# drowe67/pirip

Hardware: AMD Instinct MI355X
Metric: IQ Msamples/s demodulated (2-FSK Fs=240k Rs=10k); BER vs CPU ref (higher is better)
Workload: dtype f32; 1 GPU; BASELINE configs[1]: 2-FSK Fs=240k Rs=10k -p 24, batched synthetic u8 IQ, device-resident (fsk_demod -d equivalent); streams_per_gpu=16384

## Files before the change

include/pirip_hip.h:

```cpp
#ifndef PIRIP_HIP_H
#define PIRIP_HIP_H

#include <stddef.h>
#include <stdint.h>

#ifdef __cplusplus
extern "C" {
#endif

#define PIRIP_OK               0
#define PIRIP_ERR_BAD_ARG     (-1)
#define PIRIP_ERR_BAD_CONFIG  (-2)
#define PIRIP_ERR_NO_DEVICE   (-3)
#define PIRIP_ERR_HIP         (-4)
#define PIRIP_ERR_NOMEM       (-5)
#define PIRIP_ERR_UNSUPPORTED (-6)

#define PIRIP_IN_CU8_FSKDEMOD 0
#define PIRIP_IN_CU8_CSDR     1
#define PIRIP_IN_CS16         2
#define PIRIP_IN_CF32         3

#define PIRIP_MODE_M_MAX 4
#define PIRIP_FSK_DEFAULT_P 8
#define PIRIP_FSK_DEFAULT_NSYM 50
#define PIRIP_FDMDV_SCALE 750
#define PIRIP_STATS_PER_FRAME 10


typedef struct pirip_fsk_params {
    int Fs;
    int Rs;
    int M;
    int P;
    int Nsym;
    int est_min;
    int est_max;
    int freq_est_type;
    int tone_spacing;
    int in_format;
} pirip_fsk_params;

typedef struct pirip_fsk_info {
    int Ts, N, Nmem, Ndft, Nbits, nin_max, nstreams;
    int bytes_per_sample;
} pirip_fsk_info;

typedef struct pirip_hip_demod pirip_hip_demod;

int pirip_hip_create(const pirip_fsk_params *params, int nstreams, int device, pirip_hip_demod **out);

typedef struct pirip_fsk_recalled {
    int hann_denominator_ndft;
    float tc;
    float est_space_rs;
    float nin_threshold;
    int nin_step_div;
    float s16_scale;
    float u8d_offset;
    float u8d_scale;
    int ndft_rule;
    int sf_power;
} pirip_fsk_recalled;
void pirip_hip_recalled_defaults(pirip_fsk_recalled *r);
int pirip_hip_create_recalled(const pirip_fsk_params *params, const pirip_fsk_recalled *recalled, int nstreams, int device, pirip_hip_demod **out);
int pirip_hip_destroy(pirip_hip_demod *h);
int pirip_hip_get_info(const pirip_hip_demod *h, pirip_fsk_info *info);
#define PIRIP_KERNEL_GENERAL 0
#define PIRIP_KERNEL_WAVE 2
#define PIRIP_KERNEL_EXACT 4
#define PIRIP_KERNEL_BLOCK 3
int pirip_hip_get_kernel(const pirip_hip_demod *h);
int pirip_hip_set_exact_first_frame(pirip_hip_demod *h, int enable);
int pirip_hip_get_kernel_name(const pirip_hip_demod *h, char *buf, size_t n);
int pirip_hip_reset(pirip_hip_demod *h, void *hip_stream);
int pirip_hip_clear_estimators(pirip_hip_demod *h, void *hip_stream);

int pirip_hip_demod_batch(pirip_hip_demod *h,
                          const void *d_in, size_t in_stride_bytes, int64_t nsamp,
                          uint8_t *d_bits, size_t bits_stride,
                          float *d_rx_filt, size_t filt_stride,
                          float *d_stats, size_t stats_stride,
                          int32_t *d_nframes, int64_t *d_consumed,
                          int64_t max_frames, void *hip_stream);

typedef struct pirip_capture_report {
    int32_t segments;
    int32_t segment_frames;
    int32_t passes;
    int32_t segments_rerun;
    int64_t frames_demodulated;
} pirip_capture_report;
int pirip_hip_demod_capture(pirip_hip_demod *h, const void *d_in, int64_t nsamp, uint8_t *d_bits, float *d_rx_filt, float *d_stats,
                            int64_t max_frames, int64_t *nframes, int64_t *consumed, pirip_capture_report *report, void *hip_stream);
int pirip_hip_demod_capture_host(pirip_hip_demod *h, const void *in, int64_t nsamp, uint8_t *bits, float *rx_filt, float *stats,
                                 int64_t max_frames, int64_t *nframes, int64_t *consumed, pirip_capture_report *report);

int pirip_hip_demod_host(pirip_hip_demod *h, const void *in, int64_t nsamp,
                         uint8_t *bits, float *rx_filt, float *stats,
                         int64_t max_frames, int64_t *nframes, int64_t *consumed);
int pirip_hip_nin0(pirip_hip_demod *h);

int pirip_hip_set_bit_packing(pirip_hip_demod *h, int packed);

int pirip_hip_set_estimator_band_only(pirip_hip_demod *h, int enable);

int pirip_hip_set_burst_mode(pirip_hip_demod *h, int enable);

int pirip_hip_get_Sf(pirip_hip_demod *h, int s, float *Sf_host);
int pirip_hip_enable_eye(pirip_hip_demod *h, int enable);
int pirip_hip_get_eye(pirip_hip_demod *h, int s, int normalise, float *rx_eye, int *neyetr, int *neyesamp);
int pirip_hip_get_scalars(pirip_hip_demod *h, int s, float out8[8]);
typedef struct pirip_stream_state {
    int nin;
    float norm_rx_timing, ppm, snr_est, SNRest, EbNodB, v_est, f_est[4];
    float rx_sig_pow, rx_nse_pow;
} pirip_stream_state;
int pirip_hip_get_stream_state(pirip_hip_demod *h, int s, pirip_stream_state *out);
int pirip_hip_set_freq_est_limits(pirip_hip_demod *h, int est_min, int est_max);

typedef struct pirip_hip_decim pirip_hip_decim;

int pirip_hip_decim_create(int decimation, float transition_bw, int out_s16, int device,
                           pirip_hip_decim **out);
int pirip_hip_decim_destroy(pirip_hip_decim *d);
int pirip_hip_decim_taps(const pirip_hip_decim *d, float *taps, int *ntaps);
#define PIRIP_DECIM_EXACT   0
#define PIRIP_DECIM_FMA     1
#define PIRIP_DECIM_FMA_RAW 2
int pirip_hip_decim_set_arith(pirip_hip_decim *d, int mode);
int pirip_hip_decim_get_arith(const pirip_hip_decim *d);
int64_t pirip_hip_decim_nout(const pirip_hip_decim *d, int64_t n_in);
int pirip_hip_decim_batch(pirip_hip_decim *d, const uint8_t *d_in, size_t in_stride_bytes,
                          int64_t n_in, void *d_out, size_t out_stride_bytes, int nstreams,
                          void *hip_stream);

int pirip_hip_synth_cu8(int Fs, int Rs, int M, int nstreams,
                        const int32_t *f1_hz, int tone_spacing_hz, const int32_t *skip_samples,
                        const uint8_t *d_bits, size_t bits_stride, int64_t nsym,
                        uint8_t *d_out, size_t out_stride_bytes, int64_t nsamp,
                        float amp, float sigma, uint64_t seed, void *hip_stream);

#define PIRIP_RX_TRIAL_SYNC 0x1
#define PIRIP_RX_SYNC       0x2
#define PIRIP_RX_BITS       0x4
#define PIRIP_RX_BIT_ERRORS 0x8
#define PIRIP_LDPC_INFO_PER_CALL 10

typedef struct pirip_hip_ldpc pirip_hip_ldpc;
typedef struct pirip_ldpc_info {
    int n, k, bits_per_frame, data_bytes, nbits_per_call, max_iter, nstreams;
    char name[64];
} pirip_ldpc_info;

int pirip_hip_ldpc_create(const char *code_path, int M, int Nsym, int nstreams, int device, pirip_hip_ldpc **out);
int pirip_hip_ldpc_destroy(pirip_hip_ldpc *h);
int pirip_hip_ldpc_get_info(const pirip_hip_ldpc *h, pirip_ldpc_info *info);
int pirip_hip_ldpc_reset(pirip_hip_ldpc *h, void *hip_stream);
int pirip_hip_ldpc_get_llr_history(pirip_hip_ldpc *h, int s, uint16_t *host_llr);
int pirip_hip_ldpc_rx_batch(pirip_hip_ldpc *h, const float *d_rx_filt, size_t filt_stride, const int32_t *d_ncalls, int ncalls,
                            uint8_t *d_status, uint8_t *d_payload, int32_t *d_info, void *hip_stream);
int pirip_hip_fsk_ldpc_rx_batch(pirip_hip_demod *dem, pirip_hip_ldpc *h, const void *d_in, size_t in_stride_bytes, int64_t nsamp,
                                uint8_t *d_status, uint8_t *d_payload, int32_t *d_info, float *d_stats, size_t stats_stride,
                                int32_t *d_nframes, int64_t *d_consumed, int64_t max_frames, void *hip_stream);
int pirip_hip_fsk_ldpc_last_path(const pirip_hip_ldpc *h);
typedef struct pirip_chain_group {
    pirip_hip_demod *dem; pirip_hip_ldpc *ldpc;
    const void *d_in; uint8_t *d_status; uint8_t *d_payload; int32_t *d_info; float *d_stats; int32_t *d_nframes; int64_t *d_consumed;
} pirip_chain_group;
int pirip_hip_fsk_ldpc_rx_batch_groups(const pirip_chain_group *groups, int ngroups, size_t in_stride_bytes, int64_t nsamp, size_t stats_stride,
                                       int64_t max_frames, void *hip_stream);
int pirip_hip_ldpc_rx_host(pirip_hip_ldpc *h, const float *rx_filt, int ncalls, uint8_t *status, uint8_t *payload, int32_t *info);
int pirip_hip_ldpc_llr(pirip_hip_ldpc *h, const float *d_rx_filt, int ncalls, float *d_llr, void *hip_stream);
int pirip_hip_ldpc_decode_llr(pirip_hip_ldpc *h, const float *d_llr, int ncw, uint8_t *d_bits, int32_t *d_iter_pcc, void *hip_stream);

typedef struct pirip_hip_rx pirip_hip_rx;
int pirip_hip_rx_create(pirip_hip_demod *dem, pirip_hip_ldpc *ldpc, pirip_hip_decim *dec, int64_t block, pirip_hip_rx **out);
int pirip_hip_rx_destroy(pirip_hip_rx *rx);
int64_t pirip_hip_rx_max_frames(const pirip_hip_rx *rx);
int pirip_hip_rx_input(pirip_hip_rx *rx, void **d_block, size_t *stride_bytes);
int pirip_hip_rx_process(pirip_hip_rx *rx, uint8_t *d_bits, size_t bits_stride, float *d_rx_filt, size_t filt_stride,
                         uint8_t *d_status, uint8_t *d_payload, int32_t *d_info, float *d_stats, size_t stats_stride,
                         int32_t *d_nframes, void *hip_stream);
int pirip_hip_rx_push(pirip_hip_rx *rx, const void *d_in, size_t in_stride_bytes,
                      uint8_t *d_bits, size_t bits_stride, float *d_rx_filt, size_t filt_stride,
                      uint8_t *d_status, uint8_t *d_payload, int32_t *d_info, float *d_stats, size_t stats_stride,
                      int32_t *d_nframes, void *hip_stream);
int pirip_hip_rx_get_counters(pirip_hip_rx *rx, int64_t *consumed_total, int32_t *backlog);
int pirip_hip_rx_reset(pirip_hip_rx *rx, void *hip_stream);

typedef struct pirip_hip_chan pirip_hip_chan;
typedef struct pirip_chan_info {
    int Fs, D, ntaps, ntaps_padded, ninputs, nchan, out_s16, device;
} pirip_chan_info;
int pirip_hip_chan_create(int Fs, int decimation, float transition_bw, int out_s16, int ninputs, int nchan, const int32_t *chan_input,
                          const int32_t *chan_offset_hz, int device, pirip_hip_chan **out);
int pirip_hip_chan_destroy(pirip_hip_chan *ch);
int pirip_hip_chan_get_info(const pirip_hip_chan *ch, pirip_chan_info *info);
int pirip_hip_chan_taps(const pirip_hip_chan *ch, float *taps, int *ntaps);
int64_t pirip_hip_chan_nout(const pirip_hip_chan *ch, int64_t n_in);
int pirip_hip_chan_batch(pirip_hip_chan *ch, const uint8_t *d_in, size_t in_stride_bytes, int64_t n_in, int64_t t0,
                         void *d_out, size_t out_stride_bytes, void *hip_stream);
int pirip_hip_rx_create_chan(pirip_hip_demod *dem, pirip_hip_ldpc *ldpc, pirip_hip_chan *chan, int64_t block, pirip_hip_rx **out);

#define PIRIP_TX_CARRIER_OFF 0xFF
typedef struct pirip_hip_tx pirip_hip_tx;
typedef struct pirip_tx_info {
    int Fs, Rs, M, Ts, n, k, bits_per_frame, data_bytes, preamble_syms, frame_syms, nstreams, device;
} pirip_tx_info;
int pirip_hip_tx_create(const char *code_path, int Fs, int Rs, int M, int nstreams, int device, pirip_hip_tx **out);
int pirip_hip_tx_destroy(pirip_hip_tx *h);
int pirip_hip_tx_get_info(const pirip_hip_tx *h, pirip_tx_info *info);
int pirip_hip_tx_set_tones(pirip_hip_tx *h, const int32_t *f1_hz, int tone_spacing_hz);
int pirip_hip_tx_set_gaps(pirip_hip_tx *h, const int32_t *lead_syms, const int32_t *gap_syms);
int pirip_hip_tx_reset(pirip_hip_tx *h, void *hip_stream);
int64_t pirip_hip_tx_max_syms(const pirip_hip_tx *h, int max_rec);
int pirip_hip_tx_frame(pirip_hip_tx *h, const uint8_t *d_records, size_t rec_stride, const int32_t *d_nrec, int max_rec,
                       uint8_t *d_syms, size_t sym_stride, int64_t max_syms, int32_t *d_nsym, uint8_t *d_bits, size_t bits_stride,
                       void *hip_stream);
int pirip_hip_tx_modulate(pirip_hip_tx *h, const uint8_t *d_syms, size_t sym_stride, const int32_t *d_nsym, int64_t nsym,
                          int out_format, void *d_out, size_t out_stride_bytes, float amp, float sigma, uint64_t seed, void *hip_stream);
int pirip_hip_tx_records_to_iq(pirip_hip_tx *h, const uint8_t *d_records, size_t rec_stride, const int32_t *d_nrec, int max_rec,
                               int64_t nsym, int out_format, void *d_out, size_t out_stride_bytes, float amp, float sigma, uint64_t seed,
                               int32_t *d_nsym, void *hip_stream);

#define PIRIP_TX_REPEAT_MAX_FRAMES 100
int pirip_hip_tx_repeat_max_records(const pirip_hip_tx *h, int ncalls);
int pirip_hip_tx_repeat_records(pirip_hip_tx *h, const uint8_t *d_status, size_t status_stride, const uint8_t *d_payload, size_t payload_stride,
                                const int32_t *d_ncalls, int ncalls, int source_byte, uint8_t *d_records, size_t rec_stride, int max_rec,
                                int32_t *d_nrec, void *hip_stream);

#ifndef PIRIP_NO_CODEC2_SHIM
typedef struct { float real; float imag; } COMP;
#define MODE_M_MAX 4

struct MODEM_STATS;
struct FSK {
    int Ndft, Fs, N, Rs, Ts, Nmem, P, Nsym, Nbits, f1_tx, tone_spacing, mode;
    float tc;
    int est_min, est_max, est_space;
    float *hann_table;
    float *Sf;
    COMP phi_c[MODE_M_MAX];
    COMP *f_dc;
    void *fft_cfg;
    float norm_rx_timing;
    COMP tx_phase_c;
    float EbNodB;
    float f_est[MODE_M_MAX];
    float f2_est[MODE_M_MAX];
    int freq_est_type;
    float ppm, SNRest, v_est, rx_sig_pow, rx_nse_pow;
    int nin, burst_mode, lock_nin;
    struct MODEM_STATS *stats;
    int normalise_eye;
    void *pirip_priv;
};

// ... 114 lines not shown
```

pirip_amd/binding.py:

```python
import ctypes as C
import os
import subprocess

_HERE = os.path.dirname(os.path.abspath(__file__))
_LIB = os.environ.get("PIRIP_HIP_LIB") or os.path.join(_HERE, "lib", "libpirip_hip.so")

IN_CU8_FSKDEMOD, IN_CU8_CSDR, IN_CS16, IN_CF32 = 0, 1, 2, 3
STATS_PER_FRAME = 10


class PiripError(RuntimeError):
    pass


class FskParams(C.Structure):
    _fields_ = [("Fs", C.c_int), ("Rs", C.c_int), ("M", C.c_int), ("P", C.c_int), ("Nsym", C.c_int),
                ("est_min", C.c_int), ("est_max", C.c_int), ("freq_est_type", C.c_int),
                ("tone_spacing", C.c_int), ("in_format", C.c_int)]


class FskInfo(C.Structure):
    _fields_ = [("Ts", C.c_int), ("N", C.c_int), ("Nmem", C.c_int), ("Ndft", C.c_int), ("Nbits", C.c_int),
                ("nin_max", C.c_int), ("nstreams", C.c_int), ("bytes_per_sample", C.c_int)]

# ... 97 lines not shown
    L.pirip_hip_rx_reset.argtypes = [vp, vp]
    L.pirip_hip_rx_create_chan.argtypes = [vp, vp, vp, i64, C.POINTER(vp)]
    L.pirip_hip_chan_create.argtypes = [i32, i32, C.c_float, i32, i32, i32, vp, vp, i32, C.POINTER(vp)]
    L.pirip_hip_chan_destroy.argtypes = [vp]
    L.pirip_hip_chan_get_info.argtypes = [vp, C.POINTER(ChanInfo)]
    L.pirip_hip_chan_taps.argtypes = [vp, vp, C.POINTER(i32)]
    L.pirip_hip_chan_nout.restype = i64
    L.pirip_hip_chan_nout.argtypes = [vp, i64]
    L.pirip_hip_chan_batch.argtypes = [vp, vp, sz, i64, i64, vp, sz, vp]
    L.pirip_hip_tx_create.argtypes = [C.c_char_p, i32, i32, i32, i32, i32, C.POINTER(vp)]
    L.pirip_hip_tx_destroy.argtypes = [vp]
    L.pirip_hip_tx_get_info.argtypes = [vp, C.POINTER(TxInfo)]
    L.pirip_hip_tx_set_tones.argtypes = [vp, vp, i32]
    L.pirip_hip_tx_set_gaps.argtypes = [vp, vp, vp]
    L.pirip_hip_tx_reset.argtypes = [vp, vp]
    L.pirip_hip_tx_max_syms.restype = i64
    L.pirip_hip_tx_max_syms.argtypes = [vp, i32]
    L.pirip_hip_tx_frame.argtypes = [vp, vp, sz, vp, i32, vp, sz, i64, vp, vp, sz, vp]
    L.pirip_hip_tx_modulate.argtypes = [vp, vp, sz, vp, i64, i32, vp, sz, C.c_float, C.c_float, C.c_uint64, vp]
    L.pirip_hip_tx_records_to_iq.argtypes = [vp, vp, sz, vp, i32, i64, i32, vp, sz, C.c_float, C.c_float, C.c_uint64, vp, vp]
    L.pirip_hip_tx_repeat_max_records.argtypes = [vp, i32]
    L.pirip_hip_tx_repeat_records.argtypes = [vp, vp, sz, vp, sz, vp, i32, i32, vp, sz, i32, vp, vp]
    _lib = L
    return L


def device_count():
    return int(lib().pirip_hip_device_count())


def selftest_sqrt():
    L = lib()
    m = C.c_uint64(0)
    L.pirip_hip_selftest_sqrt.argtypes = [C.POINTER(C.c_uint64)]
    _chk(L.pirip_hip_selftest_sqrt(C.byref(m)), "pirip_hip_selftest_sqrt")
    return int(m.value)


def selftest_div():
    L = lib()
    m = C.c_uint64(0)
    L.pirip_hip_selftest_div.argtypes = [C.POINTER(C.c_uint64)]
    _chk(L.pirip_hip_selftest_div(C.byref(m)), "pirip_hip_selftest_div")
    return int(m.value)


def _chk(rc, what):
    if rc != 0:
        raise PiripError(f"{what}: {lib().pirip_hip_strerror(rc).decode()} ({rc})")


class FskRecalled(C.Structure):
    _fields_ = [("hann_denominator_ndft", C.c_int), ("tc", C.c_float), ("est_space_rs", C.c_float), ("nin_threshold", C.c_float),
                ("nin_step_div", C.c_int), ("s16_scale", C.c_float), ("u8d_offset", C.c_float), ("u8d_scale", C.c_float),
                ("ndft_rule", C.c_int), ("sf_power", C.c_int)]


def recalled(**overrides):
    r = FskRecalled()
    lib().pirip_hip_recalled_defaults(C.byref(r))
    for k, v in overrides.items():
        if k not in dict(FskRecalled._fields_):
            raise KeyError(k)
        setattr(r, k, v)
    return r


class HipDemod:

    def __init__(self, Fs, Rs, M, P=8, Nsym=50, est_min=0, est_max=0, mask=0, in_format=IN_CU8_FSKDEMOD,
                 nstreams=1, device=-1, recalled=None):
        self.L = lib()
        self.params = FskParams(Fs, Rs, M, P, Nsym, est_min, est_max, 1 if mask else 0, mask if mask else 100, in_format)
        h = C.c_void_p()
        if recalled is None:
            _chk(self.L.pirip_hip_create(C.byref(self.params), nstreams, device, C.byref(h)), "pirip_hip_create")
        else:
            rc = globals()["recalled"](**recalled)
            _chk(self.L.pirip_hip_create_recalled(C.byref(self.params), C.byref(rc), nstreams, device, C.byref(h)), "pirip_hip_create_recalled")
        self.h = h
        self.info = FskInfo()
        _chk(self.L.pirip_hip_get_info(self.h, C.byref(self.info)), "pirip_hip_get_info")
        self.nstreams = nstreams
        self.M, self.Nsym, self.Nbits, self.N = M, Nsym, self.info.Nbits, self.info.N

    def close(self):
        if getattr(self, "h", None):
            self.L.pirip_hip_destroy(self.h)
            self.h = None

    __del__ = close

    def kernel(self):
        self.L.pirip_hip_get_kernel.argtypes = [C.c_void_p]
        k = self.L.pirip_hip_get_kernel(self.h)
        return "wave" if k == 2 else "block" if k == 3 else "exact" if k == 4 else "general"

    def kernel_name(self):
        buf = C.create_string_buffer(256)
        self.L.pirip_hip_get_kernel_name.argtypes = [C.c_void_p, C.c_char_p, C.c_size_t]
        _chk(self.L.pirip_hip_get_kernel_name(self.h, buf, 256), "pirip_hip_get_kernel_name")
        return buf.value.decode()

    def reset(self, stream=0):
        _chk(self.L.pirip_hip_reset(self.h, stream), "pirip_hip_reset")

    def max_frames_for(self, nsamp):
        return nsamp // (2 * self.N - self.info.nin_max) + 2

    def demod_batch(self, d_in, in_stride, nsamp, d_bits=0, bits_stride=0, d_filt=0, filt_stride=0,
                    d_stats=0, stats_stride=0, d_nframes=0, d_consumed=0, max_frames=None, stream=0):
        if max_frames is None:
            max_frames = self.max_frames_for(nsamp)
        _chk(self.L.pirip_hip_demod_batch(self.h, d_in, in_stride, nsamp, d_bits, bits_stride, d_filt, filt_stride,
                                          d_stats, stats_stride, d_nframes, d_consumed, max_frames, stream),
             "pirip_hip_demod_batch")

    def demod_capture(self, d_in, nsamp, d_bits, d_filt=0, d_stats=0, max_frames=None, stream=0):
        if max_frames is None:
            max_frames = self.max_frames_for(nsamp)
        nf, cons, rep = C.c_int64(0), C.c_int64(0), CaptureReport()
        _chk(self.L.pirip_hip_demod_capture(self.h, d_in, nsamp, d_bits, d_filt, d_stats, max_frames, C.byref(nf), C.byref(cons),
                                            C.byref(rep), stream), "pirip_hip_demod_capture")
        return nf.value, cons.value, {k: getattr(rep, k) for k, _ in CaptureReport._fields_}

    def demod_host(self, buf, want_filt=True):
        import numpy as np
        buf = np.ascontiguousarray(buf)
        nsamp = buf.shape[0]
        maxf = self.max_frames_for(nsamp)
        fb = (self.Nbits + 7) // 8 if getattr(self, "packed", False) else self.Nbits
        bits = np.zeros((maxf, fb), dtype=np.uint8)
        filt = np.zeros((maxf, self.M * self.Nsym), dtype=np.float32)
        st = np.zeros((maxf, STATS_PER_FRAME), dtype=np.float32)
        nf, cons = C.c_int64(0), C.c_int64(0)
        _chk(self.L.pirip_hip_demod_host(self.h, buf.ctypes.data, nsamp, bits.ctypes.data,
                                         filt.ctypes.data if want_filt else None, st.ctypes.data, maxf,
                                         C.byref(nf), C.byref(cons)), "pirip_hip_demod_host")
        n = nf.value
        return {"nframes": n, "consumed": cons.value, "bits": bits[:n], "rx_filt": filt[:n] if want_filt else None,
                "stats": st[:n]}

    def set_bit_packing(self, packed=True):
        _chk(self.L.pirip_hip_set_bit_packing(self.h, 1 if packed else 0), "pirip_hip_set_bit_packing")
        self.packed = bool(packed)

    def set_exact_first_frame(self, enable=True):
        self.L.pirip_hip_set_exact_first_frame.argtypes = [C.c_void_p, C.c_int]
        _chk(self.L.pirip_hip_set_exact_first_frame(self.h, 1 if enable else 0), "pirip_hip_set_exact_first_frame")

    def set_estimator_band_only(self, enable=True):
        _chk(self.L.pirip_hip_set_estimator_band_only(self.h, 1 if enable else 0), "pirip_hip_set_estimator_band_only")

    def set_freq_est_limits(self, est_min, est_max):
        return int(self.L.pirip_hip_set_freq_est_limits(self.h, int(est_min), int(est_max)))

    def set_burst_mode(self, enable=True):
        _chk(self.L.pirip_hip_set_burst_mode(self.h, 1 if enable else 0), "pirip_hip_set_burst_mode")

    def enable_eye(self, enable=True):
        self.L.pirip_hip_enable_eye.argtypes = [C.c_void_p, C.c_int]
        _chk(self.L.pirip_hip_enable_eye(self.h, 1 if enable else 0), "pirip_hip_enable_eye")

    def eye(self, s=0, normalise=True):
        import numpy as np
        out = np.zeros((8, 160), dtype=np.float32)
        ntr, npt = C.c_int(0), C.c_int(0)
        self.L.pirip_hip_get_eye.argtypes = [C.c_void_p, C.c_int, C.c_int, C.c_void_p, C.c_void_p, C.c_void_p]
        _chk(self.L.pirip_hip_get_eye(self.h, s, 1 if normalise else 0, out.ctypes.data, C.byref(ntr), C.byref(npt)), "pirip_hip_get_eye")
        return out[:ntr.value, :npt.value].copy()

    def get_Sf(self, s=0):
        import numpy as np
        out = np.zeros(self.info.Ndft, dtype=np.float32)
        _chk(self.L.pirip_hip_get_Sf(self.h, s, out.ctypes.data), "pirip_hip_get_Sf")
        return out


class HipDecim:

    def __init__(self, D, transition_bw=0.05, out_s16=True, device=-1):
        self.L = lib()
        h = C.c_void_p()
        _chk(self.L.pirip_hip_decim_create(D, transition_bw, 1 if out_s16 else 0, device, C.byref(h)),
             "pirip_hip_decim_create")
        self.h, self.D, self.out_s16 = h, D, out_s16

    def close(self):
        if getattr(self, "h", None):
            self.L.pirip_hip_decim_destroy(self.h)
            self.h = None

    __del__ = close

    def taps(self):
        import numpy as np
        n = C.c_int(0)
        self.L.pirip_hip_decim_taps(self.h, None, C.byref(n))
        t = np.zeros(n.value, dtype=np.float32)
        self.L.pirip_hip_decim_taps(self.h, t.ctypes.data, C.byref(n))
        return t

    def nout(self, n_in):
        return int(self.L.pirip_hip_decim_nout(self.h, n_in))

    def set_arith(self, mode):
        _chk(self.L.pirip_hip_decim_set_arith(self.h, int(mode)), "pirip_hip_decim_set_arith")

    def batch(self, d_in, in_stride, n_in, d_out, out_stride, nstreams, stream=0):
        _chk(self.L.pirip_hip_decim_batch(self.h, d_in, in_stride, n_in, d_out, out_stride, nstreams, stream),
             "pirip_hip_decim_batch")


class HipChan:

    def __init__(self, Fs, D, offsets, inputs=None, transition_bw=0.05, out_s16=False, device=-1):
        import numpy as np
        self.L = lib()
        off = np.ascontiguousarray(offsets, dtype=np.int32).reshape(-1)
        inp = np.zeros(off.size, dtype=np.int32) if inputs is None else np.ascontiguousarray(inputs, dtype=np.int32).reshape(-1)
        if inp.size != off.size:
            raise ValueError("inputs and offsets must have the same length")
        ninputs = int(inp.max()) + 1 if inp.size else 1
        h = C.c_void_p()
        _chk(self.L.pirip_hip_chan_create(int(Fs), int(D), transition_bw, 1 if out_s16 else 0, ninputs, int(off.size),
                                          inp.ctypes.data if inp.size else None, off.ctypes.data if off.size else None, device, C.byref(h)),
             "pirip_hip_chan_create")
        self.h = h
        self.info = ChanInfo()
        _chk(self.L.pirip_hip_chan_get_info(self.h, C.byref(self.info)), "pirip_hip_chan_get_info")
        self.Fs, self.D, self.out_s16 = int(Fs), int(D), bool(out_s16)
        self.offsets, self.inputs = off.copy(), inp.copy()
        self.ninputs, self.nchan, self.Lp = self.info.ninputs, self.info.nchan, self.info.ntaps_padded
        self.bytes_per_sample = 4 if out_s16 else 8

    def close(self):
        if getattr(self, "h", None):
            self.L.pirip_hip_chan_destroy(self.h)
            self.h = None

    __del__ = close

    def taps(self):
        import numpy as np
        n = C.c_int(0)
        self.L.pirip_hip_chan_taps(self.h, None, C.byref(n))
        t = np.zeros(n.value, dtype=np.float32)
        self.L.pirip_hip_chan_taps(self.h, t.ctypes.data, C.byref(n))
        return t

    def nout(self, n_in):
        return int(self.L.pirip_hip_chan_nout(self.h, int(n_in)))

    def batch(self, d_in, in_stride, n_in, d_out, out_stride, t0=0, stream=0):
        _chk(self.L.pirip_hip_chan_batch(self.h, d_in, in_stride, int(n_in), int(t0), d_out, out_stride, stream), "pirip_hip_chan_batch")


TX_CARRIER_OFF = 0xFF


class HipTx:

    def __init__(self, code_path, Fs, Rs, M, nstreams=1, f1=None, shift=None, lead=0, gap=0, device=-1):
        self.L = lib()
        h = C.c_void_p()
        _chk(self.L.pirip_hip_tx_create(code_path.encode(), int(Fs), int(Rs), int(M), int(nstreams), device, C.byref(h)), "pirip_hip_tx_create")
        self.h = h
        self.info = TxInfo()
        _chk(self.L.pirip_hip_tx_get_info(self.h, C.byref(self.info)), "pirip_hip_tx_get_info")
        self.Fs, self.Rs, self.M, self.Ts, self.nstreams = int(Fs), int(Rs), int(M), self.info.Ts, int(nstreams)
        self.k, self.data_bytes, self.record_bytes = self.info.k, self.info.data_bytes, 1 + self.info.data_bytes
        self.bits_per_frame, self.frame_syms, self.preamble_syms = self.info.bits_per_frame, self.info.frame_syms, self.info.preamble_syms
        self.bps = 1 if M == 2 else 2
        if f1 is not None:
            self.set_tones(f1, shift if shift is not None else Rs)
        self.set_gaps(lead, gap)

    def close(self):
        if getattr(self, "h", None):
            self.L.pirip_hip_tx_destroy(self.h)
            self.h = None

    __del__ = close

    def _per_stream(self, v):
        import numpy as np
        a = np.ascontiguousarray(v, dtype=np.int32).reshape(-1)
        if a.size == 1:
            a = np.full(self.nstreams, int(a[0]), dtype=np.int32)
        if a.size != self.nstreams:
            raise ValueError("one value, or one per stream")
        return a

    def set_tones(self, f1, shift):
        a = self._per_stream(f1)
        _chk(self.L.pirip_hip_tx_set_tones(self.h, a.ctypes.data, int(shift)), "pirip_hip_tx_set_tones")

    def set_gaps(self, lead=0, gap=0):
        a, b = self._per_stream(lead), self._per_stream(gap)
        _chk(self.L.pirip_hip_tx_set_gaps(self.h, a.ctypes.data, b.ctypes.data), "pirip_hip_tx_set_gaps")

    def reset(self, stream=0):
        _chk(self.L.pirip_hip_tx_reset(self.h, stream), "pirip_hip_tx_reset")

    def max_syms(self, max_rec):
        return int(self.L.pirip_hip_tx_max_syms(self.h, int(max_rec)))
# ... 158 lines not shown
```

pirip_amd/csrc/demod_handle.hpp:

```cpp
#pragma once
#include <hip/hip_runtime.h>
#include <cstdint>

#include "fsk_device.hpp"
#include "fsk_plan.hpp"

struct CaptureWork;

struct pirip_hip_demod {
    pirip::FskPlan plan;
    int nstreams = 0;
    int device = 0;
    int last_hip = 0;
    int kernel = 0;
    float *d_hann = nullptr; float2 *d_tw = nullptr; uint16_t *d_perm = nullptr; float *d_lut = nullptr;
    float2 *d_tph = nullptr; int16_t *d_teeth = nullptr; uint32_t *d_mask_dtheta = nullptr;
    float2 *d_osc_drift = nullptr; float2 *d_osc_step = nullptr; float2 *d_timing_rec = nullptr; float *d_fast_tab = nullptr;
    float *d_Sf = nullptr; uint32_t *d_theta = nullptr; float2 *d_hist = nullptr; pirip::StreamScalars *d_scal = nullptr; float2 *d_phic = nullptr;
    void *d_stage_in = nullptr; size_t stage_in_bytes = 0;
    uint8_t *d_stage_bits = nullptr; float *d_stage_filt = nullptr; float *d_stage_stats = nullptr;
    int32_t *d_stage_nframes = nullptr; int64_t *d_stage_consumed = nullptr; int64_t stage_frames = 0;
    int nin0 = 0;
    bool fresh = true;
    int exact0 = 1;
    int32_t *d_first = nullptr;
    float *d_eye = nullptr;
    struct CaptureWork *capture = nullptr;
};

namespace pirip {
void demod_fill_args(const pirip_hip_demod *h, DemodArgs *a);
bool demod_bind(const pirip_hip_demod *h);
}
```

pirip_amd/csrc/fsk_demod_wave.hip:

```cpp
#include <hip/hip_runtime.h>

#include <cmath>
#include <cstdio>
#include <cstdlib>

#include "../../include/pirip_hip.h"
#include "demod_simd.hpp"
#include "fsk_device.hpp"

namespace pirip {

namespace {

constexpr int kWave = 64;

struct cf { float x, y; };

__device__ __forceinline__ float add_lane_up(float a, float b)
{
    float r;
    asm("v_add_f32_dpp %0, %1, %2 wave_shl:1 row_mask:0xf bank_mask:0xf bound_ctrl:0" : "=v"(r) : "v"(a), "v"(b));
    return r;
}

// ... 28 lines not shown

__device__ __forceinline__ v2f scale_lo(v2f h, v2f x)
{
    v2f r; asm("v_pk_mul_f32 %0, %1, %2 op_sel_hi:[0,1]" : "=v"(r) : "v"(h), "v"(x)); return r;
}
__device__ __forceinline__ v2f scale_hi(v2f h, v2f x)
{
    v2f r; asm("v_pk_mul_f32 %0, %1, %2 op_sel:[1,0] op_sel_hi:[1,1]" : "=v"(r) : "v"(h), "v"(x)); return r;
}
__device__ __forceinline__ float mag2(v2f w)
{
    v2f sq;
    asm("v_pk_mul_f32 %0, %1, %1" : "=v"(sq) : "v"(w));
    float r;
    asm("v_add_f32 %0, %1, %2" : "=v"(r) : "v"(sq.x), "v"(sq.y));
    return r;
}
__device__ __forceinline__ v2f smooth2(v2f sf, v2f mag, v2f k)
{
    v2f t;
    asm("v_pk_mul_f32 %0, %0, %3 op_sel_hi:[1,0]\n\t"
        "v_pk_mul_f32 %1, %2, %3 op_sel:[0,1] op_sel_hi:[1,1]\n\t"
        "v_pk_add_f32 %0, %0, %1"
        : "+v"(sf), "=&v"(t) : "v"(mag), "v"(k));
    return sf;
}

template <int FMT> struct InFmt;
template <> struct InFmt<PIRIP_IN_CU8_FSKDEMOD> { static constexpr int BPS = 2; static constexpr bool NEUTRAL_OK = true; static constexpr uint32_t NEUTRAL = 0x7F7F7F7Fu; };
template <> struct InFmt<PIRIP_IN_CU8_CSDR> { static constexpr int BPS = 2; static constexpr bool NEUTRAL_OK = false; static constexpr uint32_t NEUTRAL = 0x80808080u; };
template <> struct InFmt<PIRIP_IN_CS16> { static constexpr int BPS = 4; static constexpr bool NEUTRAL_OK = true; static constexpr uint32_t NEUTRAL = 0u; };
template <> struct InFmt<PIRIP_IN_CF32> { static constexpr int BPS = 8; static constexpr bool NEUTRAL_OK = true; static constexpr uint32_t NEUTRAL = 0u; };

__device__ __forceinline__ float cvt_s16(float x)
{
    const float hi = x * 0.00133514404296875f;
    return __builtin_fmaf(x, -0x1.e60f04p-20f, hi);
}
template <int FMT>
__device__ __forceinline__ v2f decode(const uint32_t *rw, int k)
{
    if (FMT == PIRIP_IN_CU8_FSKDEMOD || FMT == PIRIP_IN_CU8_CSDR) {
        const uint32_t v = rw[k >> 1];
        return cvt_u8_pair<FMT>(v2f{(k & 1) ? ubyte2(v) : ubyte0(v), (k & 1) ? ubyte3(v) : ubyte1(v)});
    } else if (FMT == PIRIP_IN_CS16) {
        const uint32_t v = rw[k];
        return v2f{cvt_s16((float)(short)(v & 0xffffu)), cvt_s16((float)((int)v >> 16))};
    } else {
        return v2f{__builtin_bit_cast(float, rw[2 * k]), __builtin_bit_cast(float, rw[2 * k + 1])};
    }
}
template <int FMT>
__device__ __forceinline__ v2f lds_sample(const unsigned char *p)
{
    if (FMT == PIRIP_IN_CU8_FSKDEMOD || FMT == PIRIP_IN_CU8_CSDR) {
        const uint32_t v = *(const uint16_t *)p;
        return cvt_u8_pair<FMT>(v2f{ubyte0(v), ubyte1(v)});
    } else if (FMT == PIRIP_IN_CS16) {
        const uint32_t v = *(const uint32_t *)p;
        return v2f{cvt_s16((float)(short)(v & 0xffffu)), cvt_s16((float)((int)v >> 16))};
    } else {
        const float2 v = *(const float2 *)p;
        return v2f{v.x, v.y};
    }
}

constexpr int cmax(int a, int b) { return a > b ? a : b; }

__device__ __forceinline__ float atan2_turns(float y, float x)
{
    const float ax = fabsf(x), ay = fabsf(y);
    const float mn = ax < ay ? ax : ay, mx = ax < ay ? ay : ax;
    const float t = mx > 0.f ? mn * __builtin_amdgcn_rcpf(mx) : 0.f;
    const float s1 = t * t, s2 = s1 * s1, s4 = s2 * s2;
    const float p01 = __builtin_fmaf(s1, -0.05304612219333649f, 0.15915483236312866f);
    const float p23 = __builtin_fmaf(s1, -0.02213626727461815f, 0.031745944172143936f);
    const float p45 = __builtin_fmaf(s1, -0.00889870710670948f, 0.015346021391451359f);
    const float p67 = __builtin_fmaf(s1, -0.0006453014793805778f, 0.0034795869141817093f);
    const float q0 = __builtin_fmaf(s2, p23, p01), q1 = __builtin_fmaf(s2, p67, p45);
    float r = __builtin_fmaf(s4, q1, q0) * t;
    r = ay > ax ? 0.25f - r : r;
    r = x < 0.f ? 0.5f - r : r;
    return __builtin_copysignf(r, y);
}

constexpr float kLlrMax = 24.0f;
__device__ __forceinline__ float ln_i0_tab(const float *tab, float x)
{
    const bool in = x < 32.0f;
    const float xs = (in ? x : 32.0f) * 8.0f;
    const int j = (int)xs;
    const float f = xs - (float)j;
    const float t0 = tab[j], t1 = tab[j + 1];
    return (t0 + (f * (t1 - t0))) + (in ? 0.0f : x - 32.0f);
}
__device__ __forceinline__ uint32_t spread16(uint32_t x)
{
    x = (x | (x << 8)) & 0x00FF00FFu; x = (x | (x << 4)) & 0x0F0F0F0Fu; x = (x | (x << 2)) & 0x33333333u; x = (x | (x << 1)) & 0x55555555u;
    return x;
}

#ifdef PIRIP_WAVE_TIMING
__device__ int g_wave_stop_phase = -1;
#define PIRIP_T_DECL long long t_acc_[8] = {0, 0, 0, 0, 0, 0, 0, 0}; long long t_last_ = __builtin_amdgcn_s_memtime(); \
    const int t_stop_ = __builtin_amdgcn_readfirstlane(g_wave_stop_phase)
#define PIRIP_T_MARK(i) { const long long t_now_ = __builtin_amdgcn_s_memtime(); t_acc_[i] += t_now_ - t_last_; t_last_ = t_now_; } \
    if (t_stop_ == (i)) { pos += nin; frame++; wave_lds_sync(); continue; } else (void)0
#else
#define PIRIP_T_DECL do { } while (0)
#define PIRIP_T_MARK(i) do { } while (0)
#endif

template <int M, int TS, int P, int NSYM, int NDFT, int FMT>
struct WaveCfg {
    static constexpr int BPS = InFmt<FMT>::BPS;
    static constexpr int N = TS * NSYM;
    static constexpr int NMEM = N + 2 * TS;
    static constexpr int Q = TS / 4;
    static constexpr int HIST = 2 * TS + Q;
    static constexpr int STEP = TS / P;
    static constexpr int NLANES = NSYM + 2;
    static constexpr int NFFT = (N - Q) / (NDFT / 2) - 1;
    static constexpr int GUARD_B = ((HIST * BPS + 15) / 16) * 16;
    static constexpr int SUP_B = (N + Q) * BPS;
    static constexpr int NDMA16 = SUP_B / 1024;
    static constexpr int NDMA4 = (SUP_B - NDMA16 * 1024 + 255) / 256;
    static constexpr bool DIRECT = FMT == PIRIP_IN_CF32 && NDFT >= 256;
    static constexpr int HEAD_B = 1024, DUMP_B = 256;
    static_assert(!DIRECT || ((TS + Q) * BPS <= HEAD_B && 3 * TS >= 2 * TS + Q), "the head holds blocks 0..2's new samples");
    static constexpr int RAW_B = DIRECT ? GUARD_B + HEAD_B + DUMP_B : GUARD_B + NDMA16 * 1024 + NDMA4 * 256;
    static constexpr int XPS256 = 16 * 17 * 8;
    static constexpr int XP_FFT_B = NDFT == 256 ? 4 * XPS256 : NDFT == 512 ? 4480 : 8 * 72 * 8;
    static constexpr int XP_B = cmax(cmax(XP_FFT_B, NDFT * 4), NDFT == 256 ? 64 * 20 * 4 : NDFT == 128 ? 8 * 136 * 4 : 0);
    static constexpr int TAIL_DW = HIST * BPS / 4;
    static constexpr int TRAILER_DW = GUARD_B / 4;
    static_assert((HIST * BPS) % 4 == 0 && (GUARD_B - HIST * BPS) % 4 == 0, "tail copies move whole dwords");
    static_assert(GUARD_B + (2 * M + 1) * 4 <= M * HIST * 8, "the state block holds the raw tail and its trailer");
    static constexpr int CHS = (BPS == 2) ? TS : (TS % 8 == 0 ? 8 : TS % 4 == 0 ? 4 : 2);
    static constexpr int CH_DW = CHS * BPS / 4;
    static_assert(TS % 2 == 0 && TS % P == 0 && P >= 4, "bad Ts / P");
    static_assert(NLANES <= kWave, "one lane per symbol block");
    static_assert((TS * BPS) % 16 == 0 && (CHS * BPS) % 16 == 0 && TS % CHS == 0, "block and chunk strides keep 16-byte alignment");
    static_assert((N + Q) / (NDFT / 2) - 1 == NFFT && N / (NDFT / 2) - 1 == NFFT, "numffts must not depend on nin");
    static_assert(NDFT == 256 ? (NFFT >= 4) : NDFT == 512 ? (NFFT % 2 == 0) : (NDFT == 128 && NFFT <= 8),
                  "FFT batches (Ndft = 256: the last batch of 4 may be partial; Ndft = 128: one batch of up to eight)");
    static_assert((NFFT - 1) * (NDFT / 2) + NDFT <= N - Q, "FFT windows stay inside the shortest frame");
    static_assert(M * P <= 48, "window prefix sums are kept in registers");
};

template <class C, int M> constexpr int wave_lds_bytes() { return C::RAW_B + C::XP_B; }

}

template <int M, int TS, int P, int NSYM, int NDFT, int FMT, int WPB, int WPS, bool FFT_FMA = false, bool MASK = false, int BAND = 0>
__global__ __launch_bounds__(kWave * WPB, WPS) void fsk_demod_wave_kernel(DemodArgs a_kernarg, int nstreams)
{
    constexpr bool INPLACE = TS == 10;
    static_assert(offsetof(DemodArgs, d) == 0, "the argument block is the first kernel argument");
    auto ap = [&]() {
        if constexpr (INPLACE) return (const __attribute__((address_space(4))) DemodArgs *)__builtin_amdgcn_kernarg_segment_ptr();
        else return (const DemodArgs *)&a_kernarg;
    }();
#define PIRIP_ARGS_REREAD() do { if constexpr (INPLACE) asm volatile("" : "+s"(ap)); } while (0)
#define a (*ap)
#define d (ap->d)
    static_assert(BAND == 0 || ((BAND == 2 || BAND == 4) && NDFT == 256 && !MASK), "band-only estimator: Ndft = 256, peak method, 32 or 64 bins");
    auto cmul = [](v2f x, v2f t) { return FFT_FMA ? rot_step(x, t) : cmul_x(x, t); };
    using C = WaveCfg<M, TS, P, NSYM, NDFT, FMT>;
    constexpr int N = C::N, NMEM = C::NMEM, HIST = C::HIST, STEP = C::STEP, Q = C::Q, BPS = C::BPS;
    constexpr int GUARD_B = C::GUARD_B;

    __shared__ __attribute__((aligned(16))) unsigned char s_raw[WPB][C::RAW_B];
    __shared__ __attribute__((aligned(16))) unsigned char s_xp[WPB][C::XP_B];
    constexpr int TAB_F = NDFT == 256 ? 12 * 16 * 4 : NDFT == 512 ? 8 * 16 * 2 + 12 * 32 * 2 : 8 * 16 * 2;
    __shared__ __attribute__((aligned(16))) float s_tab[TAB_F];
    __shared__ __attribute__((aligned(16))) float2 s_tph[P];
    __shared__ __attribute__((aligned(16))) float2 s_tgain[NSYM + 2];
    __shared__ float s_misc[WPB][3];
    extern __shared__ __attribute__((aligned(16))) float s_lnI0[];

    const int lane0 = threadIdx.x & (kWave - 1);
    const int wv = __builtin_amdgcn_readfirstlane(threadIdx.x >> 6);
    const int sid = blockIdx.x * WPB + wv;

    if (NDFT == 256) {
        for (int i = threadIdx.x; i < 12 * 16; i += kWave * WPB)
            ((float4 *)s_tab)[i] = ((const float4 *)a.t.fast_tab)[(i & 15) * 12 + (i >> 4)];
    } else {
        for (int i = threadIdx.x; i < TAB_F / 4; i += kWave * WPB) ((float4 *)s_tab)[i] = ((const float4 *)(a.t.fast_tab + NDFT))[i];
    }
    if constexpr (P <= 10) if (a.io.soft.llr) {
        if (a.io.soft.llr_map == kLlrRician) { for (int i = threadIdx.x; i < 258; i += kWave * WPB) s_lnI0[i] = a.io.soft.lnI0[i]; }
        else if (threadIdx.x < 20) {
            const int sg = threadIdx.x >> 2, cc = threadIdx.x & 3;
            const float c2 = sg == 0 ? 0.226f : sg == 1 ? 0.1245f : sg == 2 ? 0.0288f : sg == 3 ? 0.002f : 0.0f;
            const float c1 = sg == 0 ? 0.0125f : sg == 1 ? 0.2177f : sg == 2 ? 0.6314f : sg == 3 ? 0.9048f : 0.9867f;
            const float c0 = sg == 0 ? -0.0012f : sg == 1 ? -0.108f : sg == 2 ? -0.5645f : sg == 3 ? -1.2997f : -2.2053f;
            s_lnI0[threadIdx.x] = cc == 0 ? c2 : cc == 1 ? c1 : cc == 2 ? c0 : 0.0f;
        }
    }
    if (threadIdx.x < P) s_tph[threadIdx.x] = a.t.tph[threadIdx.x];
    if (threadIdx.x < NSYM + 2) s_tgain[threadIdx.x] = a.t.timing_rec[(threadIdx.x < NSYM + 1 ? threadIdx.x : 0) * P];
    __syncthreads();
    if (sid >= nstreams) return;
    if (a.io.seg && a.io.seg[sid].max_frames < 0) return;

    unsigned char *raw = s_raw[wv];
    unsigned char *xpb = s_xp[wv];

    uint32_t *st32 = (uint32_t *)(a.s.hist + (size_t)sid * M * HIST);
    int ninp = __builtin_amdgcn_readfirstlane((int)st32[C::TRAILER_DW + 2 * M]);
    uint32_t dthp[M];
    int tixp[M];
#pragma unroll
    for (int m = 0; m < M; m++) {
        dthp[m] = (uint32_t)__builtin_amdgcn_readfirstlane((int)st32[C::TRAILER_DW + m]);
        tixp[m] = __builtin_amdgcn_readfirstlane((int)st32[C::TRAILER_DW + M + m]);
    }
    for (int i = lane0; i < GUARD_B / 4; i += kWave) ((uint32_t *)raw)[i] = ninp ? st32[i] : InFmt<FMT>::NEUTRAL;

#define PIRIP_PHASE_LANE(name) int name = lane0; asm volatile("" : "+v"(name))
    constexpr int NOWN = NDFT / kWave;
    constexpr int NB = BAND ? BAND : NOWN;
    auto own_sfi = [](int ln, int b) {
        const int bin = BAND ? ((ln & 15) + 16 * b)
                      : NDFT == 256 ? ((ln & 15) + 16 * b + 64 * (ln >> 4)) : NDFT == 512 ? ((ln & 31) + 32 * (8 * (ln >> 5) + b)) : (ln + 64 * b);
        return (bin + NDFT / 2) & (NDFT - 1);
    };
    float Sf[NOWN];
    float hann16[NDFT == 256 ? 1 : 16];
    if constexpr (NDFT == 512) {
#pragma unroll
        for (int i = 0; i < 16; i++) hann16[i] = a.t.fast_tab[(lane0 & 31) + 32 * (i >> 3) + 64 * (i & 7)];
    }
    if constexpr (NDFT == 128) {
#pragma unroll
        for (int i = 0; i < 16; i++) hann16[i] = a.t.fast_tab[(lane0 & 7) + 8 * i];
    }
#pragma unroll
    for (int b = 0; b < NB; b++) Sf[b] = a.s.Sf[(size_t)sid * NDFT + own_sfi(lane0, b)];

    float sc_norm_rx_timing, sc_ppm, sc_SNRest;
    int sc_nin;
    {
        const StreamScalars sc = a.s.scal[sid];
        sc_norm_rx_timing = sc.norm_rx_timing; sc_ppm = sc.ppm; sc_SNRest = sc.SNRest; sc_nin = sc.nin;
        if (lane0 == 0) { s_misc[wv][0] = sc.snr_est; s_misc[wv][1] = sc.EbNodB; s_misc[wv][2] = sc.v_est; }
    }

    int64_t seg_in = 0, out0 = 0, max_frames = a.io.max_frames;
    if (a.io.seg) {
        const SegDesc sd = a.io.seg[sid];
        seg_in = sd.in_off; out0 = sd.out_frame0; max_frames = sd.max_frames;
    }
    const uint8_t *in_base = a.io.in + (size_t)sid * a.io.in_stride + (size_t)seg_in * BPS;
    const int64_t nsamp = a.io.nsamp - seg_in;
    const __amdgpu_buffer_rsrc_t rsrc =
        __builtin_amdgcn_make_buffer_rsrc((void *)in_base, 0, (int)(uint32_t)(BPS * nsamp), 0x00020000);

    int nin = __builtin_amdgcn_readfirstlane(sc_nin);
    int64_t pos = 0, frame = 0;
    if (a.io.first) { pos = __builtin_amdgcn_readfirstlane(a.io.first[sid]); frame = pos ? 1 : 0; }
    const int64_t frame_first = frame;
    int last_freqi0 = 0, last_freqi1 = 0, last_freqi2 = 0, last_freqi3 = 0;

    typedef __attribute__((address_space(3))) void *lds_ptr;
    auto dma_frame = [&](int64_t p0) {
        const uint32_t goff = (uint32_t)__builtin_amdgcn_readfirstlane((int)(uint32_t)(p0 * BPS));
        if constexpr (C::DIRECT) {
            __builtin_amdgcn_raw_ptr_buffer_load_lds(rsrc, (lds_ptr)(raw + GUARD_B), 16, lane0 * 16, goff, 0, 0);
#pragma unroll
            for (int i = 0; i < (C::SUP_B + 8191) / 8192; i++)
                __builtin_amdgcn_raw_ptr_buffer_load_lds(rsrc, (lds_ptr)(raw + GUARD_B + C::HEAD_B), 4, lane0 * 128, goff + i * 8192, 0, 0);
            return;
        }
#pragma unroll
        for (int i = 0; i < C::NDMA16; i++)
            __builtin_amdgcn_raw_ptr_buffer_load_lds(rsrc, (lds_ptr)(raw + GUARD_B + i * 1024), 16, lane0 * 16, goff + i * 1024, 0, 0);
#pragma unroll
        for (int i = 0; i < C::NDMA4; i++)
            __builtin_amdgcn_raw_ptr_buffer_load_lds(rsrc, (lds_ptr)(raw + GUARD_B + C::NDMA16 * 1024 + i * 256), 4, lane0 * 4,
                                                     goff + C::NDMA16 * 1024 + i * 256, 0, 0);
    };
    constexpr bool SOFT_OK = P <= 10;
    uint32_t soft_carry = 0;
    int soft_cb = 0, soft_w = 0;
    uint32_t *words_o = nullptr;
    if constexpr (SOFT_OK) if (a.io.soft.llr) { words_o = a.io.soft.words + (size_t)sid * a.io.soft.words_stride + (a.io.soft.bit0 >> 5); }
    auto soft_append = [&](uint32_t W, int nb) {
        const uint32_t merged = soft_carry | (soft_cb ? (W >> soft_cb) : W);
        if (soft_cb + nb >= 32) {
            if (lane0 == 0) words_o[soft_w] = merged;
            soft_w++;
            soft_carry = soft_cb ? (W << (32 - soft_cb)) : 0u;
            soft_cb = soft_cb + nb - 32;
        } else { soft_carry = merged; soft_cb += nb; }
    };
    constexpr int NBITS = NSYM * (M == 2 ? 1 : 2);
    wave_lds_sync();
    dma_frame(pos);
    PIRIP_T_DECL;

    while (frame < max_frames && pos + nin <= nsamp) {
        PIRIP_ARGS_REREAD();
        const int nold = NMEM - nin;
        PIRIP_T_MARK(7);
        asm volatile("s_waitcnt vmcnt(0)" ::: "memory");
        wave_lds_sync();
        PIRIP_T_MARK(0);
        const unsigned char *smp = raw + GUARD_B;
        const uint32_t goff_frame = (uint32_t)__builtin_amdgcn_readfirstlane((int)(uint32_t)(pos * BPS));
        auto fft_in = [&](const unsigned char *p) -> v2f {
            if constexpr (C::DIRECT && BPS == 8) {
                const auto v = __builtin_amdgcn_raw_buffer_load_b64(rsrc, (int)(p - smp), (int)goff_frame, 0);
                return __builtin_bit_cast(v2f, v);
            } else if constexpr (C::DIRECT) {
                const uint32_t v = (uint32_t)__builtin_amdgcn_raw_buffer_load_b32(rsrc, (int)(p - smp), (int)goff_frame, 0);
                return v2f{cvt_s16((float)(short)(v & 0xffffu)), cvt_s16((float)((int)v >> 16))};
            } else return lds_sample<FMT>(p);
        };
        const v2f ktc{d.one_minus_tc, d.tc};
        if constexpr (NDFT == 256) {
            PIRIP_PHASE_LANE(lane);
            const int grp = lane >> 4, e16 = lane & 15;
            const float4 *ftab = (const float4 *)s_tab + e16;
            constexpr int XPS = C::XPS256;
            float4 tabv[12];
#pragma unroll
            for (int i = 0; i < 12; i++) tabv[i] = ftab[16 * i];
#pragma unroll 1
            for (int bt = 0; bt < (C::NFFT + 3) / 4; bt++) {
                int jj = 4 * bt + grp;
                if (C::NFFT % 4) jj = jj < C::NFFT ? jj : C::NFFT - 1;
                const int ga = e16 >> 2, gb = e16 & 3;
                const int base = ga + 4 * gb;
                const unsigned char *src = smp + BPS * ((NDFT / 2) * jj + base);
                v2f W[16];
                v2f hann2[8];
                {
                    const float4 h0 = tabv[0], h1 = tabv[1], h2 = tabv[2], h3 = tabv[3];
                    hann2[0] = v2f{h0.x, h0.y}; hann2[1] = v2f{h0.z, h0.w}; hann2[2] = v2f{h1.x, h1.y}; hann2[3] = v2f{h1.z, h1.w};
                    hann2[4] = v2f{h2.x, h2.y}; hann2[5] = v2f{h2.z, h2.w}; hann2[6] = v2f{h3.x, h3.y}; hann2[7] = v2f{h3.z, h3.w};
                }
#pragma unroll
                for (int t = 0; t < 16; t++) {
                    const v2f x = fft_in(src + 16 * BPS * t);
                    const int c = t & 3, dd = t >> 2;
                    W[4 * c + dd] = (t & 1) ? scale_hi(hann2[t >> 1], x) : scale_lo(hann2[t >> 1], x);
                }
#pragma unroll
                for (int c = 0; c < 4; c++) bfly4(W[4 * c], W[4 * c + 1], W[4 * c + 2], W[4 * c + 3]);
                bfly4(W[0], W[4], W[8], W[12]);
#pragma unroll
                for (int k = 1; k < 4; k++) {
                    v2f f1 = cmul(W[4 + k], v2f{a.tw_s2[6 * (k - 1) + 0], a.tw_s2[6 * (k - 1) + 1]});
                    v2f f2 = cmul(W[8 + k], v2f{a.tw_s2[6 * (k - 1) + 2], a.tw_s2[6 * (k - 1) + 3]});
                    v2f f3 = cmul(W[12 + k], v2f{a.tw_s2[6 * (k - 1) + 4], a.tw_s2[6 * (k - 1) + 5]});
                    bfly4(W[k], f1, f2, f3);
                    W[4 + k] = f1; W[8 + k] = f2; W[12 + k] = f3;
                }
                {
                    float2 *xp = (float2 *)(xpb + grp * XPS);
#pragma unroll
                    for (int e = 0; e < 16; e++) xp[e16 * 17 + e] = make_float2(W[e].x, W[e].y);
                    wave_lds_sync();
#pragma unroll
                    for (int g = 0; g < 16; g++) { const float2 v = xp[g * 17 + e16]; W[g] = v2f{v.x, v.y}; }
                }
                {
                    const float4 c4 = tabv[4], c5 = tabv[5];
                    const v2f tw3[3] = {v2f{c4.x, c4.y}, v2f{c4.z, c4.w}, v2f{c5.x, c5.y}};
#pragma unroll
                    for (int aa = 0; aa < 4; aa++) {
                        v2f f1 = cmul(W[4 * aa + 1], tw3[0]);
                        v2f f2 = cmul(W[4 * aa + 2], tw3[1]);
                        v2f f3 = cmul(W[4 * aa + 3], tw3[2]);
                        bfly4(W[4 * aa], f1, f2, f3);
                        W[4 * aa + 1] = f1; W[4 * aa + 2] = f2; W[4 * aa + 3] = f3;
                    }
                }
#pragma unroll
                for (int b = 0; b < (BAND ? BAND : 4); b++) {
                    const float *trow = (const float *)(ftab);
                    auto tf = [&](int f) { const float4 c = tabv[f >> 2]; return (f & 3) == 0 ? c.x : (f & 3) == 1 ? c.y : (f & 3) == 2 ? c.z : c.w; };
                    (void)trow;
                    const v2f t1{tf(22 + 6 * b), tf(23 + 6 * b)}, t2{tf(24 + 6 * b), tf(25 + 6 * b)}, t3{tf(26 + 6 * b), tf(27 + 6 * b)};
                    v2f f1 = cmul(W[4 + b], t1);
                    v2f f2 = cmul(W[8 + b], t2);
                    v2f f3 = cmul(W[12 + b], t3);
                    bfly4(W[b], f1, f2, f3);
                    W[4 + b] = f1; W[8 + b] = f2; W[12 + b] = f3;
                }
                wave_lds_sync();
                if constexpr (BAND != 0) {
                    float m2b[BAND], rb[BAND];
                    unsigned kmin = 0xffffffffu;
#pragma unroll
                    for (int b = 0; b < BAND; b++) { m2b[b] = mag2(W[b]); kmin = umin2(kmin, fbits(m2b[b])); }
                    if (__all(kmin >= kSqrtLo)) {
#pragma unroll
                        for (int b = 0; b < BAND; b++) rb[b] = sqrt_rn_normal<FMT != PIRIP_IN_CF32, true>(m2b[b]);
                    } else {
                        kmin = 0xffffffffu;
#pragma unroll
                        for (int b = 0; b < BAND; b++) kmin = umin2(kmin, sqrt_key(m2b[b]));
                        if (__all(kmin >= kSqrtLo - 1u)) {
#pragma unroll
                            for (int b = 0; b < BAND; b++) rb[b] = sqrt_rn_normal<FMT != PIRIP_IN_CF32>(m2b[b]);
                        } else {
#pragma unroll
                            for (int b = 0; b < BAND; b++) rb[b] = sqrtf(m2b[b]);
                        }
                    }
                    float2 *mx = (float2 *)xpb;
#pragma unroll
                    for (int b = 0; b < BAND; b += 2) mx[(b / 2) * 64 + lane] = make_float2(rb[b], rb[b + 1]);
                    wave_lds_sync();
                    float2 rt[BAND / 2][4];
#pragma unroll
                    for (int b = 0; b < BAND; b += 2)
#pragma unroll
                        for (int g2 = 0; g2 < 4; g2++) rt[b / 2][g2] = mx[(b / 2) * 64 + g2 * 16 + e16];
#pragma unroll
                    for (int b = 0; b < BAND; b += 2) {
                        v2f sp{Sf[b], Sf[b + 1]};
#pragma unroll
                        for (int g2 = 0; g2 < 4; g2++)
                            if (C::NFFT % 4 == 0 || 4 * bt + g2 < C::NFFT) sp = smooth2(sp, v2f{rt[b / 2][g2].x, rt[b / 2][g2].y}, ktc);
                        Sf[b] = sp.x; Sf[b + 1] = sp.y;
                    }
                    wave_lds_sync();
                } else {
                    float *mx = (float *)xpb;
                    float4 *row = (float4 *)(mx + lane * 20);
#pragma unroll
                    for (int q4 = 0; q4 < 4; q4++)
                        row[q4] = make_float4(mag2(W[4 * q4 + 0]), mag2(W[4 * q4 + 1]), mag2(W[4 * q4 + 2]), mag2(W[4 * q4 + 3]));
                    wave_lds_sync();
                    float4 m2[4];
                    unsigned kmin = 0xffffffffu;
#pragma unroll
                    for (int g2 = 0; g2 < 4; g2++) {
                        m2[g2] = *(const float4 *)(mx + (g2 * 16 + e16) * 20 + 4 * grp);
                        kmin = umin3(umin3(kmin, fbits(m2[g2].x), fbits(m2[g2].y)), fbits(m2[g2].z), fbits(m2[g2].w));
                    }
                    float4 rt[4];
                    if (__all(kmin >= kSqrtLo)) {
#pragma unroll
                        for (int g2 = 0; g2 < 4; g2++)
                            rt[g2] = make_float4(sqrt_rn_normal<FMT != PIRIP_IN_CF32, true>(m2[g2].x), sqrt_rn_normal<FMT != PIRIP_IN_CF32, true>(m2[g2].y),
                                                 sqrt_rn_normal<FMT != PIRIP_IN_CF32, true>(m2[g2].z), sqrt_rn_normal<FMT != PIRIP_IN_CF32, true>(m2[g2].w));
                    } else {
                        kmin = 0xffffffffu;
#pragma unroll
                        for (int g2 = 0; g2 < 4; g2++)
                            kmin = umin3(umin3(kmin, sqrt_key(m2[g2].x), sqrt_key(m2[g2].y)), sqrt_key(m2[g2].z), sqrt_key(m2[g2].w));
                        if (__all(kmin >= kSqrtLo - 1u)) {
#pragma unroll
                            for (int g2 = 0; g2 < 4; g2++)
                                rt[g2] = make_float4(sqrt_rn_normal<FMT != PIRIP_IN_CF32>(m2[g2].x), sqrt_rn_normal<FMT != PIRIP_IN_CF32>(m2[g2].y),
                                                     sqrt_rn_normal<FMT != PIRIP_IN_CF32>(m2[g2].z), sqrt_rn_normal<FMT != PIRIP_IN_CF32>(m2[g2].w));
                        } else {
#pragma unroll
                            for (int g2 = 0; g2 < 4; g2++) {
                                rt[g2] = make_float4(sqrtf(m2[g2].x), sqrtf(m2[g2].y), sqrtf(m2[g2].z), sqrtf(m2[g2].w));
                                __builtin_amdgcn_sched_barrier(0);
                            }
                        }
                    }
                    {
                        v2f s01{Sf[0], Sf[1]}, s23{Sf[2], Sf[3]};
#pragma unroll
                        for (int g2 = 0; g2 < 4; g2++) {
                            if (C::NFFT % 4 == 0 || 4 * bt + g2 < C::NFFT) {
                                s01 = smooth2(s01, v2f{rt[g2].x, rt[g2].y}, ktc);
                                s23 = smooth2(s23, v2f{rt[g2].z, rt[g2].w}, ktc);
                            }
                        }
                        Sf[0] = s01.x; Sf[1] = s01.y; Sf[2] = s23.x; Sf[3] = s23.y;
                    }
                    wave_lds_sync();
                }
            }
        } else if constexpr (NDFT == 128) {
            PIRIP_PHASE_LANE(lane);
            const int f8 = lane >> 3, l8 = lane & 7;
            const int jj = f8 < C::NFFT ? f8 : C::NFFT - 1;
            const float2 *s_p2 = (const float2 *)s_tab;
            float2 *xf = (float2 *)xpb + f8 * 72;
            v2f V[16];
            {
                const unsigned char *src = smp + BPS * ((NDFT / 2) * jj + l8);
#pragma unroll
                for (int u = 0; u < 2; u++) {
                    v2f S[8];
                    {
                        v2f Wt[8];
#pragma unroll
                        for (int t = 0; t < 8; t++) {
                            const int y = u + 2 * (t & 3) + 8 * (t >> 2);
                            const v2f x = fft_in(src + BPS * 8 * y);
                            const float hn = hann16[y];
                            Wt[t] = v2f{hn * x.x, hn * x.y};
                        }
#pragma unroll
                        for (int q2 = 0; q2 < 4; q2++) { S[2 * q2] = Wt[q2] + Wt[q2 + 4]; S[2 * q2 + 1] = Wt[q2] - Wt[q2 + 4]; }
                    }
                    bfly4(S[0], S[2], S[4], S[6]);
                    {
                        v2f f1 = cmul(S[3], v2f{a.tw_s2[0], a.tw_s2[1]});
                        v2f f2 = cmul(S[5], v2f{a.tw_s2[2], a.tw_s2[3]});
                        v2f f3 = cmul(S[7], v2f{a.tw_s2[4], a.tw_s2[5]});
                        bfly4(S[1], f1, f2, f3);
                        S[3] = f1; S[5] = f2; S[7] = f3;
                    }
                    if (u == 1) wave_lds_sync();
                    float2 *wr = xf + l8 * 9;
#pragma unroll
                    for (int r = 0; r < 8; r++) wr[r] = make_float2(S[r].x, S[r].y);
                    wave_lds_sync();
#pragma unroll
                    for (int q0 = 0; q0 < 4; q0++)
#pragma unroll
                        for (int ql = 0; ql < 2; ql++) { const float2 v = xf[(q0 + 4 * ql) * 9 + l8]; V[4 * q0 + 2 * u + ql] = v2f{v.x, v.y}; }
                }
            }
            {
                const float2 t1 = s_p2[l8 * 16 + 0], t2 = s_p2[l8 * 16 + 1], t3 = s_p2[l8 * 16 + 2];
#pragma unroll
                for (int q0 = 0; q0 < 4; q0++) {
                    v2f f1 = cmul(V[4 * q0 + 1], v2f{t1.x, t1.y});
                    v2f f2 = cmul(V[4 * q0 + 2], v2f{t2.x, t2.y});
                    v2f f3 = cmul(V[4 * q0 + 3], v2f{t3.x, t3.y});
                    bfly4(V[4 * q0], f1, f2, f3);
                    V[4 * q0 + 1] = f1; V[4 * q0 + 2] = f2; V[4 * q0 + 3] = f3;
                }
            }
#pragma unroll
            for (int j1 = 0; j1 < 4; j1++) {
                const float2 t1 = s_p2[l8 * 16 + 3 + 3 * j1], t2 = s_p2[l8 * 16 + 4 + 3 * j1], t3 = s_p2[l8 * 16 + 5 + 3 * j1];
                v2f f1 = cmul(V[4 + j1], v2f{t1.x, t1.y});
                v2f f2 = cmul(V[8 + j1], v2f{t2.x, t2.y});
                v2f f3 = cmul(V[12 + j1], v2f{t3.x, t3.y});
                bfly4(V[j1], f1, f2, f3);
                V[4 + j1] = f1; V[8 + j1] = f2; V[12 + j1] = f3;
            }
            wave_lds_sync();
            {
                float *mx = (float *)xpb;
#pragma unroll
                for (int i = 0; i < 16; i++) mx[f8 * 136 + l8 + 8 * i] = mag2(V[i]);
                wave_lds_sync();
                float A[C::NFFT], B[C::NFFT];
                unsigned kmin = 0xffffffffu;
#pragma unroll
                for (int j = 0; j < C::NFFT; j++) {
                    A[j] = mx[j * 136 + lane]; B[j] = mx[j * 136 + lane + 64];
                    kmin = umin3(kmin, fbits(A[j]), fbits(B[j]));
                }
                if (__all(kmin >= kSqrtLo)) {
#pragma unroll
                    for (int j = 0; j < C::NFFT; j++) { A[j] = sqrt_rn_normal<FMT != PIRIP_IN_CF32, true>(A[j]); B[j] = sqrt_rn_normal<FMT != PIRIP_IN_CF32, true>(B[j]); }
                } else {
                    kmin = 0xffffffffu;
#pragma unroll
                    for (int j = 0; j < C::NFFT; j++) kmin = umin3(kmin, sqrt_key(A[j]), sqrt_key(B[j]));
                    if (__all(kmin >= kSqrtLo - 1u)) {
#pragma unroll
                        for (int j = 0; j < C::NFFT; j++) { A[j] = sqrt_rn_normal<FMT != PIRIP_IN_CF32>(A[j]); B[j] = sqrt_rn_normal<FMT != PIRIP_IN_CF32>(B[j]); }
                    } else {
#pragma unroll
                        for (int j = 0; j < C::NFFT; j++) { A[j] = sqrtf(A[j]); B[j] = sqrtf(B[j]); __builtin_amdgcn_sched_barrier(0); }
                    }
                }
                v2f sp{Sf[0], Sf[1]};
#pragma unroll
                for (int j = 0; j < C::NFFT; j++) sp = smooth2(sp, v2f{A[j], B[j]}, ktc);
                Sf[0] = sp.x; Sf[1] = sp.y;
                wave_lds_sync();
            }
        } else {
            PIRIP_PHASE_LANE(lane);
            const int hh = lane >> 5, L5 = lane & 31;
            const float2 *s_p2 = (const float2 *)s_tab;
            const float2 *s_p3 = (const float2 *)(s_tab + 8 * 16 * 2);
            const int q0w = L5 & 3, q1w = (L5 >> 2) & 3, q2w = L5 >> 4;
            const int q0r = L5 >> 3, r2 = L5 & 7;
            float2 *x1 = (float2 *)xpb + hh * 280;
            float2 *x2 = (float2 *)xpb + hh * 160;
#pragma unroll 1
            for (int bt = 0; bt < C::NFFT / 2; bt++) {
                const int jj = 2 * bt + hh;
                const unsigned char *src = smp + BPS * ((NDFT / 2) * jj + L5);
                v2f V[16];
#pragma unroll
                for (int u = 0; u < 2; u++) {
                    v2f S[8];
                    {
                        v2f Wt[8];
#pragma unroll
                        for (int t = 0; t < 8; t++) {
                            const v2f x = fft_in(src + BPS * (32 * u + 64 * t));
                            const float hn = hann16[8 * u + t];
                            Wt[t] = v2f{hn * x.x, hn * x.y};
                        }
#pragma unroll
                        for (int q3 = 0; q3 < 4; q3++) { S[2 * q3] = Wt[q3] + Wt[q3 + 4]; S[2 * q3 + 1] = Wt[q3] - Wt[q3 + 4]; }
                    }
                    bfly4(S[0], S[2], S[4], S[6]);
                    {
                        v2f f1 = cmul(S[3], v2f{a.tw_s2[0], a.tw_s2[1]});
                        v2f f2 = cmul(S[5], v2f{a.tw_s2[2], a.tw_s2[3]});
                        v2f f3 = cmul(S[7], v2f{a.tw_s2[4], a.tw_s2[5]});
                        bfly4(S[1], f1, f2, f3);
                        S[3] = f1; S[5] = f2; S[7] = f3;
                    }
                    if (u == 1) wave_lds_sync();
                    {
                        float2 *wr = x1 + (q0w * 9 + q1w * 2 + q2w) * 8;
#pragma unroll
                        for (int r = 0; r < 8; r++) wr[r ^ q1w] = make_float2(S[r].x, S[r].y);
                    }
                    wave_lds_sync();
#pragma unroll
                    for (int q1 = 0; q1 < 4; q1++)
#pragma unroll
                        for (int q2l = 0; q2l < 2; q2l++) {
                            const float2 v = x1[(q0r * 9 + q1 * 2 + q2l) * 8 + (r2 ^ q1)];
                            V[4 * q1 + 2 * u + q2l] = v2f{v.x, v.y};
                        }
                }
                {
                    const float2 t1 = s_p2[r2 * 16 + 0], t2 = s_p2[r2 * 16 + 1], t3 = s_p2[r2 * 16 + 2];
// ... 351 lines not shown
                    if (low_sample >= 0) { lo[m].x = lane_up(lo[m].x); lo[m].y = lane_up(lo[m].y); }
                    if (high_sample >= 0) { hi[m].x = lane_up(hi[m].x); hi[m].y = lane_up(hi[m].y); }
                }
            }
            float tmax[M];
            float sum = 0.f;
#pragma unroll
            for (int m = 0; m < M; m++) {
                v2f t;
                t.x = (1 - fract) * lo[m].x; t.y = (1 - fract) * lo[m].y;
                t.x = t.x + fract * hi[m].x; t.y = t.y + fract * hi[m].y;
                tmax[m] = (t.x * t.x) + (t.y * t.y);
                sum += tmax[m];
            }
            float mx = tmax[0]; int sym = 0;
#pragma unroll
            for (int m = 1; m < M; m++) if (tmax[m] > mx) { mx = tmax[m]; sym = m; }
            const bool act = lane < NSYM;
            if (bits_o && !d.pack_bits) {
                if (act) {
                    if (M == 2) bits_o[lane] = sym == 1;
                    else { bits_o[2 * lane + 1] = sym & 1; bits_o[2 * lane] = (sym & 2) >> 1; }
                }
            } else if (bits_o) {
                const unsigned long long mlo = __ballot(act && (sym & 1)), mhi = __ballot(act && (sym & 2));
                if (lane < frame_bytes) {
                    unsigned byte = 0;
                    if (M == 2) {
                        byte = __builtin_bitreverse32((unsigned)(mlo >> (8 * lane)) & 0xffu) >> 24;
                    } else {
                        const unsigned h4 = (unsigned)(mhi >> (4 * lane)) & 0xfu, l4 = (unsigned)(mlo >> (4 * lane)) & 0xfu;
#pragma unroll
                        for (int q = 0; q < 4; q++) byte |= (((h4 >> q) & 1u) << (7 - 2 * q)) | (((l4 >> q) & 1u) << (6 - 2 * q));
                    }
                    bits_o[lane] = (uint8_t)byte;
                }
            }
            if (act && filt_o) {
#pragma unroll
                for (int m = 0; m < M; m++) filt_o[m * NSYM + lane] = sqrtf(tmax[m]);
            }
            if constexpr (SOFT_OK) if (a.io.soft.llr) {
                float mag[M], sum2 = 0.f, mx2 = 0.f;
                unsigned kmin = 0xffffffffu, kmax = 0u;
#pragma unroll
                for (int m = 0; m < M; m++) { kmin = umin2(kmin, sqrt_key(tmax[m])); kmax = kmax > fbits(tmax[m]) ? kmax : fbits(tmax[m]); }
                const bool quick = __all(!act || (kmin >= 0x0f800000u - 1u && kmax <= kQuickHi));
                float ssig, snse;
                if (quick) {
#pragma unroll
                    for (int m = 0; m < M; m++) { mag[m] = sqrt_rn_normal<FMT != PIRIP_IN_CF32>(tmax[m]); const float p2 = mag[m] * mag[m]; sum2 = sum2 + p2; mx2 = p2 > mx2 ? p2 : mx2; }
                    ssig = wave_sum(act ? mx2 : 0.f); snse = wave_sum(act ? div_rn_const<M - 1>(sum2 - mx2) : 0.f);
                    ssig = div_rn_const<NSYM>(ssig);
                    snse = div_rn_const<NSYM>(snse) + 1e-12f;
                } else {
#pragma unroll
                    for (int m = 0; m < M; m++) { mag[m] = sqrtf(tmax[m]); const float p2 = mag[m] * mag[m]; sum2 = sum2 + p2; mx2 = p2 > mx2 ? p2 : mx2; }
                    ssig = wave_sum(act ? mx2 : 0.f); snse = wave_sum(act ? (sum2 - mx2) / (float)(M - 1) : 0.f);
                    ssig = ssig / (float)NSYM;
                    snse = (snse / (float)NSYM) + 1e-12f;
                }
                const int llr_map = a.io.soft.llr_map;
                const float g = llr_frame_gain_quick(llr_map, ssig, snse);
                float L[M];
                if (llr_map == kLlrRician) {
#pragma unroll
                    for (int m = 0; m < M; m++) L[m] = ln_i0_tab(s_lnI0, g * mag[m]);
                } else {
#pragma unroll
                    for (int m = 0; m < M; m++) {
                        const float x = g * mag[m];
                        int sg = x >= 1.0f ? 1 : 0;
                        sg = x >= 2.0f ? 2 : sg; sg = x >= 5.0f ? 3 : sg; sg = x >= 20.0f ? 4 : sg;
                        const float4 cf = ((const float4 *)s_lnI0)[sg];
                        L[m] = (((cf.x * x) * x) + (cf.y * x)) + cf.z;
                    }
                }
                float l0, l1 = 0.f;
                if (M == 2) l0 = L[0] - L[M - 1];
                else {
                    l0 = (L[0] > L[1] ? L[0] : L[1]) - (L[M - 2] > L[M - 1] ? L[M - 2] : L[M - 1]);
                    l1 = (L[0] > L[M - 2] ? L[0] : L[M - 2]) - (L[1] > L[M - 1] ? L[1] : L[M - 1]);
                }
                const float lmax = llr_map == kLlrRician ? kLlrMax : kLlrMaxUpstream;
                l0 = l0 > lmax ? lmax : (l0 < -lmax ? -lmax : l0);
                l1 = l1 > lmax ? lmax : (l1 < -lmax ? -lmax : l1);
                const _Float16 h0v = (_Float16)l0, h1v = (_Float16)l1;
                l0 = (float)h0v; l1 = (float)h1v;
                uint16_t *llr_o = a.io.soft.llr + (size_t)sid * a.io.soft.llr_stride + a.io.soft.bit0 + (size_t)frame * NBITS;
                if (act) {
                    if (M == 2) llr_o[lane] = __builtin_bit_cast(uint16_t, h0v);
                    else *(uint32_t *)(llr_o + 2 * lane) = (uint32_t)__builtin_bit_cast(uint16_t, h0v) | ((uint32_t)__builtin_bit_cast(uint16_t, h1v) << 16);
                }
                const unsigned long long h0 = __ballot(act && l0 < 0.0f), h1 = __ballot(act && l1 < 0.0f);
                if (M == 2) {
                    soft_append(__builtin_bitreverse32((uint32_t)h0), 32);
                    soft_append(__builtin_bitreverse32((uint32_t)(h0 >> 32)), NBITS - 32);
                } else {
#pragma unroll
                    for (int j = 0; j < (NBITS + 31) / 32; j++) {
                        const uint32_t z = spread16((uint32_t)(h0 >> (16 * j)) & 0xffffu) | (spread16((uint32_t)(h1 >> (16 * j)) & 0xffffu) << 1);
                        soft_append(__builtin_bitreverse32(z), (j + 1) * 32 <= NBITS ? 32 : NBITS - 32 * j);
                    }
                }
            }
            const bool last_frame = (frame + 1 >= max_frames) || (pos + nin + nin_next > nsamp);
            if (stats_o || last_frame) {
                float sig = act ? mx : 0.f, nse = act ? (sum - mx) / (float)(M - 1) : 0.f;
                sig = wave_sum(sig); nse = wave_sum(nse) + 1e-12f;
                sig = sig / (float)NSYM; nse = nse / (float)NSYM;
                sc_SNRest = sig / nse;
                float mean_e = wave_sum(act ? sqrtf(mx) : 0.f), std_e = wave_sum(act ? mx : 0.f);
                mean_e = mean_e / (float)NSYM;
                std_e = (std_e / (float)NSYM) - (mean_e * mean_e);
                std_e = std_e > 0.0f ? sqrtf(std_e) : 0.0f;
                const float EbNodB = -6.0f + (20.0f * log10f((1e-6f + mean_e) / (1e-6f + std_e)));
                if (lane == 0) {
                    s_misc[wv][0] = (0.5f * s_misc[wv][0]) + (0.5f * EbNodB);
                    s_misc[wv][1] = EbNodB;
                    s_misc[wv][2] = sqrtf(sig - nse);
                    a.s.scal[sid].rx_sig_pow = sig; a.s.scal[sid].rx_nse_pow = nse;
                    if (stats_o) { stats_o[8] = sig; stats_o[9] = nse; }
                }
            }
        } else {
            for (int i = lane; i < frame_bytes; i += kWave) if (bits_o) bits_o[i] = 0;
            for (int i = lane; i < M * NSYM; i += kWave) if (filt_o) filt_o[i] = 0.f;
            if (stats_o && lane == 0) { stats_o[8] = 0.f; stats_o[9] = 0.f; }
            if constexpr (SOFT_OK) if (a.io.soft.llr) {
                uint16_t *llr_o = a.io.soft.llr + (size_t)sid * a.io.soft.llr_stride + a.io.soft.bit0 + (size_t)frame * NBITS;
                for (int i = lane; i < NBITS; i += kWave) llr_o[i] = 0;
                for (int j = 0; j < (NBITS + 31) / 32; j++) soft_append(0u, (j + 1) * 32 <= NBITS ? 32 : NBITS - 32 * j);
            }
        }
        if constexpr (MASK) last_freqi0 = bb;
        else { last_freqi0 = freqi[0]; last_freqi1 = freqi[M > 1 ? 1 : 0]; last_freqi2 = freqi[M > 2 ? 2 : 0]; last_freqi3 = freqi[M > 3 ? 3 : 0]; }
        if (stats_o && lane == 0) {
            stats_o[0] = f_est[0]; stats_o[1] = f_est[1]; stats_o[2] = f_est[2]; stats_o[3] = f_est[3];
            stats_o[4] = sc_norm_rx_timing; stats_o[5] = sc_SNRest; stats_o[6] = (float)nin_next; stats_o[7] = sc_ppm;
        }
        PIRIP_T_MARK(5);
        pos += nin;
        nin = __builtin_amdgcn_readfirstlane(nin_next);
        frame++;
        wave_lds_sync();
    }

    if constexpr (SOFT_OK) if (words_o && soft_cb > 0 && lane0 == 0) words_o[soft_w] = soft_carry;
    asm volatile("s_waitcnt vmcnt(0)" ::: "memory");
#ifdef PIRIP_WAVE_TIMING
    if (a.io.stats && lane0 == 0 && sid == nstreams / 2)
        for (int i = 0; i < 8; i++) a.io.stats[(size_t)sid * a.io.stats_stride + i] = (float)t_acc_[i];
#endif
#pragma unroll
    for (int b = 0; b < NB; b++) if (!BAND || lane0 < 16) a.s.Sf[(size_t)sid * NDFT + own_sfi(lane0, b)] = Sf[b];
    wave_lds_sync();
    for (int i = lane0; i < GUARD_B / 4; i += kWave) st32[i] = ((const uint32_t *)raw)[i];
    const int lane = lane0;
    if (lane == 0) {
#pragma unroll
        for (int m = 0; m < M; m++) { st32[C::TRAILER_DW + m] = dthp[m]; st32[C::TRAILER_DW + M + m] = (uint32_t)tixp[m]; }
        st32[C::TRAILER_DW + 2 * M] = (uint32_t)ninp;
        StreamScalars sc = a.s.scal[sid];
        sc.nin = nin; sc.norm_rx_timing = sc_norm_rx_timing; sc.ppm = sc_ppm; sc.SNRest = sc_SNRest;
        sc.snr_est = s_misc[wv][0]; sc.EbNodB = s_misc[wv][1]; sc.v_est = s_misc[wv][2];
        if (frame > frame_first) {
            const int fq[4] = {last_freqi0, last_freqi1, last_freqi2, last_freqi3};
            for (int m = 0; m < kMaxTones; m++) {
                if (MASK) sc.f_est[m] = m < M ? (float)((fq[0] - NDFT / 2) * d.Fs / NDFT) + (float)(m * d.tone_spacing) : 0.f;
                else sc.f_est[m] = m < M ? (float)fq[m] * d.bin_hz : 0.f;
            }
        }
        a.s.scal[sid] = sc;
        if (a.io.nframes) a.io.nframes[sid] = (int32_t)frame;
        if (a.io.consumed) a.io.consumed[sid] = pos;
    }
#undef a
#undef d
#undef PIRIP_ARGS_REREAD
}

namespace {
__global__ void sqrt_selftest_kernel(unsigned long long *bad, unsigned lo, unsigned hi)
{
    unsigned long long c = 0;
    const unsigned stride = gridDim.x * blockDim.x;
    for (unsigned long long b = (unsigned long long)lo + blockIdx.x * blockDim.x + threadIdx.x; b <= hi; b += stride) {
        const float x = __builtin_bit_cast(float, (unsigned)b);
        const float want = (float)sqrt((double)x);
        if (__builtin_bit_cast(unsigned, sqrt_rn_normal<true>(x)) != __builtin_bit_cast(unsigned, want)) c++;
        if (x != 0.0f && __builtin_bit_cast(unsigned, sqrt_rn_normal<true, true>(x)) != __builtin_bit_cast(unsigned, want)) c++;
        if (__builtin_bit_cast(unsigned, sqrt_rn_normal<false>(x)) != __builtin_bit_cast(unsigned, want)) c += 1ull << 32;
    }
    if (c) atomicAdd(bad, c);
}
}

hipError_t selftest_sqrt(unsigned long long *mismatches)
{
    unsigned long long *d = nullptr;
    hipError_t e = hipMalloc(&d, sizeof(*d));
    if (e != hipSuccess) return e;
    e = hipMemset(d, 0, sizeof(*d));
    if (e == hipSuccess) {
        hipLaunchKernelGGL(sqrt_selftest_kernel, dim3(4096), dim3(256), 0, 0, d, 0u, 0u);
        hipLaunchKernelGGL(sqrt_selftest_kernel, dim3(4096), dim3(256), 0, 0, d, 0x0f800000u, 0x7f7fffffu);
        e = hipMemcpy(mismatches, d, sizeof(*d), hipMemcpyDeviceToHost);
        if (e == hipSuccess) e = hipGetLastError();
    }
    (void)hipFree(d);
    return e;
}

namespace {
template <int C>
__global__ void div_selftest_kernel(unsigned long long *bad, unsigned lo, unsigned hi)
{
    unsigned long long c = 0;
    const unsigned stride = gridDim.x * blockDim.x;
    for (unsigned long long b = (unsigned long long)lo + blockIdx.x * blockDim.x + threadIdx.x; b <= hi; b += stride) {
        const float x = __builtin_bit_cast(float, (unsigned)b);
        if (__builtin_bit_cast(unsigned, div_rn_const<C>(x)) != __builtin_bit_cast(unsigned, x / (float)C)) c++;
    }
    if (c) atomicAdd(bad, c);
}
}

hipError_t selftest_div(unsigned long long *mismatches)
{
    unsigned long long *d = nullptr;
    hipError_t e = hipMalloc(&d, 2 * sizeof(*d));
    if (e != hipSuccess) return e;
    e = hipMemset(d, 0, 2 * sizeof(*d));
    if (e == hipSuccess) {
        hipLaunchKernelGGL(div_selftest_kernel<3>, dim3(4096), dim3(256), 0, 0, d, 0u, 0x7f7fffffu);
        hipLaunchKernelGGL(div_selftest_kernel<50>, dim3(4096), dim3(256), 0, 0, d + 1, 0u, 0u);
        hipLaunchKernelGGL(div_selftest_kernel<50>, dim3(4096), dim3(256), 0, 0, d + 1, 0x01000000u, 0x7f7fffffu);
        unsigned long long h[2] = {0, 0};
        e = hipMemcpy(h, d, sizeof(h), hipMemcpyDeviceToHost);
        if (e == hipSuccess) e = hipGetLastError();
        const unsigned long long a = h[0] > 0xffffffffull ? 0xffffffffull : h[0], b = h[1] > 0xffffffffull ? 0xffffffffull : h[1];
        *mismatches = (b << 32) | a;
    }
    (void)hipFree(d);
    return e;
}

namespace {

struct WaveInst {
    int M, Ts, P, Nsym, Ndft, fmt, fft_fma, mask, wpb, wps, band;
    hipError_t (*launch)(const DemodArgs &, int, hipStream_t);
};

template <int M, int TS, int P, int NSYM, int NDFT, int FMT, int WPB, int WPS, bool FMA, bool MASK, int BAND = 0>
hipError_t launch_inst(const DemodArgs &a, int nstreams, hipStream_t stream)
{
    const dim3 g((nstreams + WPB - 1) / WPB), b(kWave * WPB);
    const size_t dyn = a.io.soft.llr ? 258 * sizeof(float) : 0;
#ifdef PIRIP_WAVE_TIMING
    {
        const char *e = getenv("PIRIP_WAVE_STOP");
        const int stop = e ? atoi(e) : -1;
        (void)hipMemcpyToSymbolAsync(HIP_SYMBOL(g_wave_stop_phase), &stop, sizeof(int), 0, hipMemcpyHostToDevice, stream);
        (void)hipStreamSynchronize(stream);
    }
#endif
    hipLaunchKernelGGL((fsk_demod_wave_kernel<M, TS, P, NSYM, NDFT, FMT, WPB, WPS, FMA, MASK, BAND>), g, b, dyn, stream, a, nstreams);
    return hipGetLastError();
}

#define PIRIP_WAVE_INST(M, TS, P, NDFT, FMT, WPB, WPS) {M, TS, P, 50, NDFT, FMT, 0, 0, WPB, WPS, 0, launch_inst<M, TS, P, 50, NDFT, FMT, WPB, WPS, false, false>}
#define PIRIP_WAVE_INST_FMA(M, TS, P, NDFT, FMT, WPB, WPS) {M, TS, P, 50, NDFT, FMT, 1, 0, WPB, WPS, 0, launch_inst<M, TS, P, 50, NDFT, FMT, WPB, WPS, true, false>}
#define PIRIP_WAVE_INST_MASK(M, TS, P, NDFT, FMT, WPB, WPS) {M, TS, P, 50, NDFT, FMT, 0, 1, WPB, WPS, 0, launch_inst<M, TS, P, 50, NDFT, FMT, WPB, WPS, false, true>}
#define PIRIP_WAVE_INST_BAND(M, TS, P, NDFT, FMT, WPB, WPS, B) {M, TS, P, 50, NDFT, FMT, 0, 0, WPB, WPS, B, launch_inst<M, TS, P, 50, NDFT, FMT, WPB, WPS, false, false, B>}
const WaveInst kInst[] = {
    PIRIP_WAVE_INST(2, 24, 24, 256, PIRIP_IN_CU8_FSKDEMOD, 4, 3),
    PIRIP_WAVE_INST_FMA(2, 24, 24, 256, PIRIP_IN_CU8_FSKDEMOD, 4, 3),
    PIRIP_WAVE_INST(2, 24, 24, 256, PIRIP_IN_CU8_CSDR, 4, 3),
    PIRIP_WAVE_INST_BAND(2, 24, 24, 256, PIRIP_IN_CU8_FSKDEMOD, 4, 3, 2), PIRIP_WAVE_INST_BAND(2, 24, 24, 256, PIRIP_IN_CU8_CSDR, 4, 3, 2),
    PIRIP_WAVE_INST_BAND(4, 24, 8, 256, PIRIP_IN_CU8_FSKDEMOD, 4, 3, 4), PIRIP_WAVE_INST_BAND(4, 24, 8, 256, PIRIP_IN_CU8_CSDR, 4, 3, 4),
#define PIRIP_TS24(M, P, WPB, WPS) \
    PIRIP_WAVE_INST(M, 24, P, 256, PIRIP_IN_CU8_FSKDEMOD, WPB, WPS), PIRIP_WAVE_INST(M, 24, P, 256, PIRIP_IN_CU8_CSDR, WPB, WPS), \
    PIRIP_WAVE_INST_MASK(M, 24, P, 256, PIRIP_IN_CU8_FSKDEMOD, WPB, WPS), PIRIP_WAVE_INST_MASK(M, 24, P, 256, PIRIP_IN_CU8_CSDR, WPB, WPS)
    PIRIP_TS24(2, 8, 4, 3), PIRIP_TS24(2, 6, 4, 3), PIRIP_TS24(4, 8, 4, 3), PIRIP_TS24(4, 6, 4, 3),
#undef PIRIP_TS24
#define PIRIP_TS40(M, P) \
    PIRIP_WAVE_INST(M, 40, P, 512, PIRIP_IN_CS16, 4, 2), PIRIP_WAVE_INST(M, 40, P, 512, PIRIP_IN_CF32, 4, ((M) == 2 ? 3 : 2)), \
    PIRIP_WAVE_INST_MASK(M, 40, P, 512, PIRIP_IN_CS16, 4, 2), PIRIP_WAVE_INST_MASK(M, 40, P, 512, PIRIP_IN_CF32, 4, ((M) == 2 ? 3 : 2))
    PIRIP_TS40(2, 8), PIRIP_TS40(2, 10), PIRIP_TS40(4, 8), PIRIP_TS40(4, 10),
#undef PIRIP_TS40
    PIRIP_WAVE_INST(2, 20, 10, 256, PIRIP_IN_CF32, 4, 3), PIRIP_WAVE_INST_MASK(2, 20, 10, 256, PIRIP_IN_CF32, 4, 3),
    PIRIP_WAVE_INST(4, 20, 10, 256, PIRIP_IN_CF32, 4, 3), PIRIP_WAVE_INST_MASK(4, 20, 10, 256, PIRIP_IN_CF32, 4, 3),
    PIRIP_WAVE_INST(2, 18, 9, 256, PIRIP_IN_CF32, 4, 3), PIRIP_WAVE_INST_MASK(2, 18, 9, 256, PIRIP_IN_CF32, 4, 3),
    PIRIP_WAVE_INST(4, 18, 9, 256, PIRIP_IN_CF32, 4, 3), PIRIP_WAVE_INST_MASK(4, 18, 9, 256, PIRIP_IN_CF32, 4, 3),
    PIRIP_WAVE_INST(2, 10, 10, 128, PIRIP_IN_CF32, 4, 4), PIRIP_WAVE_INST_MASK(2, 10, 10, 128, PIRIP_IN_CF32, 4, 4),
    PIRIP_WAVE_INST(4, 10, 10, 128, PIRIP_IN_CF32, 2, 2), PIRIP_WAVE_INST_MASK(4, 10, 10, 128, PIRIP_IN_CF32, 2, 2),
    PIRIP_WAVE_INST(2, 8, 8, 128, PIRIP_IN_CF32, 4, 4), PIRIP_WAVE_INST_MASK(2, 8, 8, 128, PIRIP_IN_CF32, 4, 4),
    PIRIP_WAVE_INST(4, 8, 8, 128, PIRIP_IN_CF32, 2, 2), PIRIP_WAVE_INST_MASK(4, 8, 8, 128, PIRIP_IN_CF32, 2, 2),
};
#undef PIRIP_WAVE_INST
#undef PIRIP_WAVE_INST_FMA
#undef PIRIP_WAVE_INST_MASK
#undef PIRIP_WAVE_INST_BAND

const WaveInst *find_inst(const FskDims &d)
{
    if (!d.recalled_fast_ok) return nullptr;
    for (const WaveInst &w : kInst)
        if (w.M == d.M && w.Ts == d.Ts && w.P == d.P && w.Nsym == d.Nsym && w.Ndft == d.Ndft && w.fmt == d.in_format && w.fft_fma == d.fft_fma &&
            w.mask == (d.freq_est_type != 0) && w.band == d.est_band) return &w;
    return nullptr;
}

}

bool demod_wave_applicable(const FskDims &d) { return find_inst(d) != nullptr; }

int demod_wave_streams_per_cu(const FskDims &d) { const WaveInst *w = find_inst(d); return w ? 4 * w->wps : 0; }

bool demod_wave_soft_capable(const FskDims &d) { return find_inst(d) != nullptr && d.P <= 10 && d.Nsym == 50; }

int demod_wave_describe(const FskDims &d, char *buf, size_t n)
{
    const WaveInst *w = find_inst(d);
    if (!w) return 0;
    static const char *const fmt_name[] = {"u8 -d", "u8 csdr", "s16", "f32"};
    return snprintf(buf, n, "fsk_demod_wave_kernel<M=%d,Ts=%d,P=%d,Nsym=%d,Ndft=%d,%s,%s%s%d streams/block,%d waves/SIMD>", w->M, w->Ts, w->P, w->Nsym,
                    w->Ndft, fmt_name[w->fmt & 3], w->mask ? "mask estimator," : w->band ? "band-only estimator," : "", w->fft_fma ? "fused FFT multiply," : "", w->wpb, w->wps);
}

int64_t demod_wave_max_samples(const FskDims &d)
{
    const int bps = d.in_format == PIRIP_IN_CF32 ? 8 : d.in_format == PIRIP_IN_CS16 ? 4 : 2;
    return 0x7fffff00LL / bps * 2 / 2;
}

hipError_t launch_demod_wave(const DemodArgs &a, int nstreams, hipStream_t stream)
{
    const WaveInst *w = find_inst(a.d);
    if (!w || a.io.nsamp > demod_wave_max_samples(a.d)) return hipErrorNotSupported;
    return w->launch(a, nstreams, stream);
}

}
```

pirip_amd/csrc/fsk_device.hpp:

```cpp
#pragma once
#include <hip/hip_runtime.h>
#include <cstdint>

#include "fsk_plan.hpp"

namespace pirip {

constexpr int kEyeTraces = 8, kEyePoints = 160;

struct StreamScalars {
    int32_t nin;
    float norm_rx_timing;
    float ppm;
    float snr_est;
    float SNRest;
    float EbNodB;
    float v_est;
    float f_est[kMaxTones];
    float rx_sig_pow;
    float rx_nse_pow;
};

struct DemodTables {
    const float *hann;
    const float2 *tw;
    const uint16_t *perm;
    const float *lut;
    const float2 *tph;
    const int16_t *teeth;
    const uint32_t *mask_dtheta;
    const float2 *osc_drift;
    const float2 *osc_step;
    const float2 *timing_rec;
    const float *fast_tab;
};

struct DemodState {
    float *Sf;
    uint32_t *theta;
    float2 *hist;
    StreamScalars *scal;
    float2 *phic;
};

struct SoftOut {
    uint16_t *llr; size_t llr_stride;
    uint32_t *words; size_t words_stride;
    const float *lnI0;
    int bit0;
    int llr_map;
};

constexpr int kLlrUpstream = 0, kLlrRician = 1;
constexpr float kLlrMaxUpstream = 1000.0f;
__device__ __forceinline__ float logbesseli0_upstream(float x)
{
    float c2 = 0.226f, c1 = 0.0125f, c0 = -0.0012f;
    if (x >= 1.0f) { c2 = 0.1245f; c1 = 0.2177f; c0 = -0.108f; }
    if (x >= 2.0f) { c2 = 0.0288f; c1 = 0.6314f; c0 = -0.5645f; }
    if (x >= 5.0f) { c2 = 0.002f; c1 = 0.9048f; c0 = -1.2997f; }
    if (x >= 20.0f) { c2 = 0.0f; c1 = 0.9867f; c0 = -2.2053f; }
    return (((c2 * x) * x) + (c1 * x)) + c0;
}
template <int C>
__device__ __forceinline__ float div_rn_const(float x)
{
    if constexpr (C == 1) return x;
    constexpr float c = (float)C, rc = 1.0f / c;
    const float q = x * rc;
    return __builtin_fmaf(__builtin_fmaf(-q, c, x), rc, q);
}
__device__ __forceinline__ float llr_frame_gain(int llr_map, float sig, float nse)
{
    const float a2 = sig - nse;
    const float amp = a2 > 0.f ? sqrtf(a2) : 0.f;
    if (llr_map == kLlrRician) return (2.0f * amp) / nse;
    return amp > 0.f ? (2.0f * (sig / nse)) / amp : 0.f;
}

struct SegDesc {
    int64_t in_off;
    int64_t out_frame0;
    int32_t max_frames;
    int32_t reserved;
};

struct DemodIO {
    const uint8_t *in; size_t in_stride; int64_t nsamp;
    uint8_t *bits; size_t bits_stride;
    float *filt; size_t filt_stride;
    float *stats; size_t stats_stride;
    int32_t *nframes; int64_t *consumed;
    int64_t max_frames;
    SoftOut soft;
    const SegDesc *seg;
    float *eye;
    const int32_t *first;
    int32_t *first_out;
    int exact0_fmt;
};

struct DemodArgs {
    FskDims d;
    FftStage stages[kMaxStages];
    DemodTables t;
    DemodState s;
    DemodIO io;
    float tw_s2[18];
};

int demod_batch_seg(pirip_hip_demod *h, const void *d_in, size_t in_stride_bytes, int64_t nsamp, uint8_t *d_bits, size_t bits_stride,
                    float *d_rx_filt, size_t filt_stride, float *d_stats, size_t stats_stride, int32_t *d_nframes, int64_t *d_consumed,
                    int64_t max_frames, const SegDesc *seg, hipStream_t st);
int fsk_ldpc_rx_batch_seg(pirip_hip_demod *dem, pirip_hip_ldpc *h, const void *d_in, size_t in_stride_bytes, int64_t nsamp,
                          uint8_t *d_status, uint8_t *d_payload, int32_t *d_info, float *d_stats, size_t stats_stride,
                          int32_t *d_nframes, int64_t *d_consumed, int64_t max_frames, const SegDesc *seg, hipStream_t st);
int ldpc_handle_shape(const pirip_hip_ldpc *h, int *M, int *Nsym, int *nstreams, int *device);
int demod_batch_soft(pirip_hip_demod *h, const void *d_in, size_t in_stride_bytes, int64_t nsamp, const SoftOut &so, float *d_stats, size_t stats_stride,
                     int32_t *d_nframes, int64_t *d_consumed, int64_t max_frames, hipStream_t st, int s0 = 0, int n = -1,
                     const SegDesc *seg = nullptr);
int demod_handle_shape(const pirip_hip_demod *h, int *M, int *Nsym, int *nstreams, int *device);
int demod_streams_per_cu(const pirip_hip_demod *h);
bool demod_soft_capable(const pirip_hip_demod *h, int64_t nsamp);

size_t demod_general_lds_bytes(const FskDims &d);
hipError_t launch_demod_general(const DemodArgs &a, int nstreams, hipStream_t stream);
bool demod_exact0_applicable(const FskDims &d);
hipError_t launch_demod_exact0(const DemodArgs &a, int nstreams, hipStream_t stream);
bool demod_exact_applicable(const FskDims &d);
hipError_t launch_demod_exact(const DemodArgs &a, int nstreams, hipStream_t stream);
hipError_t selftest_atan2(const float *d_y, const float *d_x, float *d_out, int n);
bool demod_wave_applicable(const FskDims &d);
int demod_wave_describe(const FskDims &d, char *buf, size_t n);
int demod_wave_streams_per_cu(const FskDims &d);
bool demod_wave_soft_capable(const FskDims &d);
int64_t demod_wave_max_samples(const FskDims &d);
hipError_t launch_demod_wave(const DemodArgs &a, int nstreams, hipStream_t stream);
bool demod_block_applicable(const FskDims &d);
int demod_block_describe(const FskDims &d, char *buf, size_t n);
hipError_t launch_demod_block(const DemodArgs &a, int nstreams, hipStream_t stream);
inline hipError_t launch_demod_kind(int kind, const DemodArgs &a, int nstreams, hipStream_t stream)
{
    return kind == 2 ? launch_demod_wave(a, nstreams, stream) : kind == 3 ? launch_demod_block(a, nstreams, stream) :
           kind == 4 ? launch_demod_exact(a, nstreams, stream) : launch_demod_general(a, nstreams, stream);
}
const char *demod_wave_source_hash();
hipError_t selftest_sqrt(unsigned long long *mismatches);
hipError_t selftest_div(unsigned long long *mismatches);

}
```

pirip_amd/csrc/fsk_plan.cpp:

```cpp
#include "fsk_plan.hpp"

#include <cassert>
#include <cmath>
#include <cstdlib>
#include <cstring>
#include <string>

#include "../../include/pirip_hip.h"

namespace pirip {

namespace {
struct cf { float re, im; };
inline cf cmul(cf a, cf b) { return {a.re * b.re - a.im * b.im, a.re * b.im + a.im * b.re}; }
}

int FskPlan::init(int Fs, int Rs, int M, int P, int Nsym, int est_min, int est_max,
                  int freq_est_type, int tone_spacing, int in_format, const pirip_fsk_recalled *recalled)
{
    pirip_fsk_recalled rc;
    recalled_defaults(&rc);
    const pirip_fsk_recalled dflt = rc;
    if (recalled) rc = *recalled;
    if (!(rc.tc > 0.0f && rc.tc <= 1.0f) || !(rc.est_space_rs >= 0.0f) || !(rc.nin_threshold > 0.0f && rc.nin_threshold < 0.5f) || rc.nin_step_div < 2 ||
// ... 26 lines not shown
    d.one_minus_tc = 1 - d.tc;
    d.nin_step = d.Ts / rc.nin_step_div;
    d.nin_thresh = rc.nin_threshold;
    d.s16_scale = rc.s16_scale;
    d.sf_power = rc.sf_power;
    d.u8_table = (in_format == PIRIP_IN_CU8_FSKDEMOD && (rc.u8d_offset != dflt.u8d_offset || rc.u8d_scale != dflt.u8d_scale)) ? 1 : 0;
    d.recalled_fast_ok = (rc.nin_threshold == dflt.nin_threshold && rc.nin_step_div == dflt.nin_step_div && rc.s16_scale == dflt.s16_scale &&
                          !d.u8_table && rc.ndft_rule == dflt.ndft_rule && rc.sf_power == dflt.sf_power) ? 1 : 0;
    d.freq_est_type = freq_est_type ? 1 : 0;
    d.tone_spacing = tone_spacing;
    d.in_format = in_format;
    d.hist_len = 2 * d.Ts + d.nin_step;
    {
        const int step = d.Ts / P;
        auto gcd = [](int a, int b) { while (b) { const int t = a % b; a = b; b = t; } return a; };
        d.grp = gcd(gcd(step, d.nin_step > 0 ? d.nin_step : step), d.hist_len);
        if (d.grp < 1) d.grp = 1;
    }
    d.burst_mode = 0;
    d.block_stagger = 0;
    d.fft_fma = 0;
    d.est_band = 0;
    d.pack_bits = 0;
    d.bin_hz = (float)Fs / (float)Ndft;

    const int est_space = rc.est_space_rs * Rs;
    if (!fsk_est_range(Fs, Ndft, est_min, est_max, &d.est_st, &d.est_en)) return PIRIP_ERR_BAD_CONFIG;
    d.f_zero = (est_space * Ndft) / Fs;

    hann.resize(Ndft);
    {
        const float w = rc.hann_denominator_ndft ? (2 * M_PI) / ((float)Ndft) : (2 * M_PI) / ((float)Ndft - 1);
        cf dphi{cosf(w), sinf(w)};
        cf rphi{.5f, 0.0f};
        rphi = cmul(cf{dphi.re, -dphi.im}, rphi);
        for (int i = 0; i < Ndft; i++) {
            rphi = cmul(dphi, rphi);
            hann[i] = .5f - rphi.re;
        }
    }

    twiddle.resize(2 * (size_t)Ndft);
    for (int i = 0; i < Ndft; i++) {
        const double pi = 3.141592653589793238462643383279502884197169399375105820974944;
        double phase = -2 * pi * i / Ndft;
        twiddle[2 * i] = (float)std::cos(phase);
        twiddle[2 * i + 1] = (float)std::sin(phase);
    }

    int radices[kMaxStages], ms[kMaxStages], nst = 0;
    {
        int n = Ndft;
        while (n > 1) {
            int p = (n % 4 == 0) ? 4 : 2;
            n /= p;
            radices[nst] = p; ms[nst] = n; nst++;
        }
    }
    d.nstages = nst;
    {
        int fs = 1;
        int fstr[kMaxStages];
        for (int l = 0; l < nst; l++) { fstr[l] = fs; fs *= radices[l]; }
        for (int l = 0; l < nst; l++) {
            int src = nst - 1 - l;
            stages[l] = FftStage{radices[src], ms[src], fstr[src]};
        }
        leaf_perm.resize(Ndft);
        for (int n = 0; n < Ndft; n++) {
            int rem = n, idx = 0;
            for (int l = 0; l < nst; l++) {
                int q = rem / ms[l]; rem -= q * ms[l];
                idx += q * fstr[l];
            }
            leaf_perm[n] = (uint16_t)idx;
        }
        leaf_iperm.resize(Ndft);
        for (int n = 0; n < Ndft; n++) leaf_iperm[leaf_perm[n]] = (uint16_t)n;
    }

    u8_lut.resize(256);
    for (int x = 0; x < 256; x++) {
        if (in_format == PIRIP_IN_CU8_CSDR) u8_lut[x] = ((float)x) / (255 / 2.0) - 1.0;
        else u8_lut[x] = ((float)x - (double)rc.u8d_offset) / (double)rc.u8d_scale;
    }

    timing_ph.resize(2 * (size_t)P);
    for (int k = 0; k < P; k++) {
        timing_ph[2 * k] = (float)std::cos(2.0 * M_PI * k / P);
        timing_ph[2 * k + 1] = (float)std::sin(2.0 * M_PI * k / P);
    }

    teeth.clear();
    mask_dtheta.assign(kMaxTones, 0u);
    d.mask_len = 0; d.n_teeth = 0;
    if (d.freq_est_type) {
        if (tone_spacing <= 0) return PIRIP_ERR_BAD_CONFIG;
        std::vector<uint8_t> mask(Ndft, 0);
        for (int i = 0; i < 3; i++) mask[i] = 1;
        int bin = 0;
        for (int m = 1; m <= M - 1; m++) {
            bin = (int)(std::round((double)((float)m * tone_spacing * Ndft / Fs)) - 1);
            for (int i = bin; i <= bin + 2; i++) if (i >= 0 && i < Ndft) mask[i] = 1;
        }
        d.mask_len = bin + 2 + 1;
        for (int i = 0; i < d.mask_len && i < Ndft; i++) if (mask[i]) teeth.push_back((int16_t)i);
        d.n_teeth = (int)teeth.size();
        mask_dtheta.assign((size_t)Ndft * M, 0u);
    }
    if (teeth.empty()) teeth.push_back(0);

    {
        const int per = d.freq_est_type ? M : 1;
        osc_drift.assign(2 * (size_t)Ndft * per, 0.f);
        osc_step.assign(2 * (size_t)Ndft * per, 0.f);
        for (int b = 0; b < Ndft; b++) {
            for (int m = 0; m < per; m++) {
                float f_est; double ideal_turns;
                if (d.freq_est_type) {
                    const float foff = (float)((b - Ndft / 2) * Fs / Ndft);
                    f_est = foff + (float)(m * tone_spacing);
                    ideal_turns = 0.0;
                } else {
                    f_est = (float)(b - Ndft / 2) * d.bin_hz;
                    ideal_turns = (double)(b - Ndft / 2) / Ndft;
                }
                const float w = 2 * M_PI * ((f_est) / (float)(Fs));
                const float c = cosf(w), s = sinf(w);
                if (d.freq_est_type) {
                    double turns = std::atan2((double)s, (double)c) / (2.0 * M_PI);
                    turns -= std::floor(turns);
                    const uint32_t step = (uint32_t)((uint64_t)std::llround(turns * 4294967296.0) & 0xffffffffull);
                    mask_dtheta[(size_t)b * M + m] = step;
                    ideal_turns = (double)step / 4294967296.0;
                }
                const double a = std::sqrt((double)c * c + (double)s * s) - 1.0;
                double dd = std::atan2((double)s, (double)c) - 2.0 * M_PI * ideal_turns;
                dd -= 2.0 * M_PI * std::round(dd / (2.0 * M_PI));
                const size_t ix = 2 * ((size_t)b * per + m);
                osc_drift[ix] = (float)a; osc_drift[ix + 1] = (float)dd;
                osc_step[ix] = c; osc_step[ix + 1] = s;
            }
        }
        timing_rec.resize(2 * (size_t)d.nint);
        const float wt = 2 * M_PI * ((float)(Rs) / (float)(P * Rs));
        cf dph{cosf(wt), sinf(wt)}, ph{1.0f, 0.0f};
        for (int i = 0; i < d.nint; i++) {
            timing_rec[2 * i] = ph.re; timing_rec[2 * i + 1] = ph.im;
            ph = cmul(ph, dph);
        }
    }
    fast_tab.clear();
    for (auto &v : tw_s2) v = 0.f;
    if (Ndft == 256) {
        fast_tab.assign(16 * 48, 0.f);
        for (int e = 0; e < 16; e++) {
            float *row = &fast_tab[(size_t)e * 48];
            const int a = e >> 2, b = e & 3, base = a + 4 * b;
            for (int t = 0; t < 16; t++) row[t] = hann[base + 16 * t];
            for (int r = 1; r <= 3; r++) {
                row[16 + 2 * (r - 1)] = twiddle[2 * (4 * e * r)];
                row[16 + 2 * (r - 1) + 1] = twiddle[2 * (4 * e * r) + 1];
            }
            for (int bp = 0; bp < 4; bp++)
                for (int r = 1; r <= 3; r++) {
                    const int k = (e + 16 * bp) * r;
                    row[22 + 2 * (3 * bp + (r - 1))] = twiddle[2 * k];
                    row[22 + 2 * (3 * bp + (r - 1)) + 1] = twiddle[2 * k + 1];
                }
        }
        for (int k = 1; k <= 3; k++)
            for (int r = 1; r <= 3; r++) {
                tw_s2[2 * (3 * (k - 1) + (r - 1))] = twiddle[2 * (16 * k * r)];
                tw_s2[2 * (3 * (k - 1) + (r - 1)) + 1] = twiddle[2 * (16 * k * r) + 1];
            }
    }
    if (Ndft == 512) {
        fast_tab.assign(512 + 8 * 16 * 2 + 12 * 32 * 2, 0.f);
        for (int i = 0; i < 512; i++) fast_tab[i] = hann[i];
        float *p2 = &fast_tab[512];
        for (int r2 = 0; r2 < 8; r2++) {
            for (int j = 1; j <= 3; j++) {
                p2[2 * (r2 * 16 + (j - 1))] = twiddle[2 * (16 * r2 * j)];
                p2[2 * (r2 * 16 + (j - 1)) + 1] = twiddle[2 * (16 * r2 * j) + 1];
            }
            for (int j2 = 0; j2 < 4; j2++)
                for (int j = 1; j <= 3; j++) {
                    const int k = 4 * (r2 + 8 * j2) * j;
                    p2[2 * (r2 * 16 + 3 + 3 * j2 + (j - 1))] = twiddle[2 * k];
                    p2[2 * (r2 * 16 + 3 + 3 * j2 + (j - 1)) + 1] = twiddle[2 * k + 1];
                }
        }
        float *p3 = &fast_tab[512 + 8 * 16 * 2];
        for (int jj = 0; jj < 4; jj++)
            for (int j = 1; j <= 3; j++)
                for (int L = 0; L < 32; L++) {
                    const int k = (L + 32 * jj) * j;
                    p3[2 * ((3 * jj + (j - 1)) * 32 + L)] = twiddle[2 * k];
                    p3[2 * ((3 * jj + (j - 1)) * 32 + L) + 1] = twiddle[2 * k + 1];
                }
        for (int j = 1; j <= 3; j++) { tw_s2[2 * (j - 1)] = twiddle[2 * (64 * j)]; tw_s2[2 * (j - 1) + 1] = twiddle[2 * (64 * j) + 1]; }
    }
    if (Ndft == 128) {
        fast_tab.assign(128 + 8 * 16 * 2, 0.f);
        for (int i = 0; i < 128; i++) fast_tab[i] = hann[i];
        float *p2 = &fast_tab[128];
        for (int r = 0; r < 8; r++) {
            for (int j = 1; j <= 3; j++) {
                p2[2 * (r * 16 + (j - 1))] = twiddle[2 * (4 * r * j)];
                p2[2 * (r * 16 + (j - 1)) + 1] = twiddle[2 * (4 * r * j) + 1];
            }
            for (int j1 = 0; j1 < 4; j1++)
                for (int j = 1; j <= 3; j++) {
                    const int k = (r + 8 * j1) * j;
                    p2[2 * (r * 16 + 3 + 3 * j1 + (j - 1))] = twiddle[2 * k];
                    p2[2 * (r * 16 + 3 + 3 * j1 + (j - 1)) + 1] = twiddle[2 * k + 1];
                }
        }
        for (int j = 1; j <= 3; j++) { tw_s2[2 * (j - 1)] = twiddle[2 * (16 * j)]; tw_s2[2 * (j - 1) + 1] = twiddle[2 * (16 * j) + 1]; }
    }
    if (Ndft == 4096) {
        fast_tab.assign(16 * 256 * 2, 0.f);
        for (int i = 0; i < 15; i++)
            for (int t = 0; t < 256; t++) {
                const int k4 = i < 3 ? 0 : (i - 3) / 3, r = i < 3 ? i + 1 : (i - 3) % 3 + 1;
                const int k = i < 3 ? 4 * t * r : (t + 256 * k4) * r;
                fast_tab[2 * (i * 256 + t)] = twiddle[2 * k]; fast_tab[2 * (i * 256 + t) + 1] = twiddle[2 * k + 1];
            }
    }
    return PIRIP_OK;
}

bool fsk_est_range(int Fs, int Ndft, int est_min, int est_max, int *st_out, int *en_out)
{
    if (est_min == 0 && est_max == 0) { est_min = 0; est_max = Fs; }
    else if (est_min < -Fs / 2 || est_max > Fs / 2 || est_max <= est_min) return false;
    int st = (est_min * Ndft) / Fs + Ndft / 2; if (st < 0) st = 0;
    int en = (est_max * Ndft) / Fs + Ndft / 2; if (en > Ndft) en = Ndft;
    *st_out = st; *en_out = en;
    return true;
}

void FskMod::init(int Fs_, int Rs_, int M_, int f1, int spacing)
{
    Fs = Fs_; Rs = Rs_; M = M_; Ts = Fs_ / Rs_; f1_tx = f1; tone_spacing = spacing;
    ph_re = cosf(0); ph_im = sinf(0);
}

void FskMod::mod(const uint8_t *bits, int nbits, float *out, bool complex_out)
{
    cf dosc[kMaxTones];
    for (int m = 0; m < M; m++) {
        const float w = 2 * M_PI * ((float)(f1_tx + (tone_spacing * m)) / (float)(Fs));
        dosc[m] = cf{cosf(w), sinf(w)};
    }
    const int bps = (M == 2) ? 1 : 2;
    const int nsym = nbits / bps;
    cf ph{ph_re, ph_im};
    int bit_i = 0;
    for (int i = 0; i < nsym; i++) {
        int sym = 0;
        for (int b = 0; b < bps; b++) sym = (sym << 1) | (bits[bit_i++] == 1 ? 1 : 0);
        const cf dph = dosc[sym];
        for (int j = 0; j < Ts; j++) {
            ph = cmul(ph, dph);
            if (complex_out) { out[2 * (i * Ts + j)] = 2 * ph.re; out[2 * (i * Ts + j) + 1] = 2 * ph.im; }
            else out[i * Ts + j] = 2 * ph.re;
        }
    }
    const float av = sqrtf((ph.re * ph.re) + (ph.im * ph.im));
    ph_re = ph.re / av; ph_im = ph.im / av;
}

void test_frame_bits(uint8_t *frame, int framesize)
{
    srand(158324);
    for (int i = 0; i < framesize; i++) frame[i] = rand() & 0x1;
}

void PutBits::init(int framesize_, float valid_thresh_)
{
    framesize = framesize_; valid_thresh = valid_thresh_;
    tx.resize(framesize); rx.assign(framesize, 0);
    test_frame_bits(tx.data(), framesize);
    bitcnt = biterr = 0; packetcnt = 0;
}

bool PutBits::push(uint8_t bit, int *errs_out)
{
    rx[framesize - 1] = bit;
    int errs = 0;
    for (int i = 0; i < framesize; i++) errs += rx[i] != tx[i];
    bool valid = errs < valid_thresh * framesize;
    if (valid) { packetcnt++; bitcnt += framesize; biterr += errs; }
    std::memmove(rx.data(), rx.data() + 1, framesize - 1);
    if (errs_out) *errs_out = errs;
    return valid;
}

#define CSDR_PI ((float)3.14159265358979323846)
int csdr_filter_len(float transition_bw)
{
    int result = 4.0 / transition_bw;
    if (result % 2 == 0) result++;
    return result;
}
// ... 73 lines not shown
```

pirip_amd/csrc/fsk_plan.hpp:

```cpp
#pragma once
#include <cstdint>
#include <vector>

#include "../../include/pirip_hip.h"

namespace pirip {

constexpr int kMaxTones = 4;
constexpr int kMaxStages = 16;

struct FftStage { int radix; int m; int fstride; };

struct FskDims {
    int Fs, Rs, M, P, Nsym;
    int Ts, N, Nmem, Ndft, Nbits, nint;
    int est_st, est_en, f_zero;
    int freq_est_type;
    int tone_spacing;
    int mask_len;
    int n_teeth;
    int in_format;
    int hist_len;
    int grp;
    int nstages;
    int pack_bits;
    int burst_mode;
    int fft_fma;
    int est_band;
    float tc, one_minus_tc;
    float bin_hz;
    int nin_step;
    float nin_thresh;
    float s16_scale;
    int u8_table;
    int sf_power;
    int recalled_fast_ok;
    int block_stagger;
};

struct FskPlan {
    FskDims d{};
    FftStage stages[kMaxStages]{};
    std::vector<float> hann;
    std::vector<float> twiddle;
    std::vector<uint16_t> leaf_perm;
    std::vector<uint16_t> leaf_iperm;
    std::vector<float> u8_lut;
    std::vector<float> timing_ph;
    std::vector<int16_t> teeth;
    std::vector<uint32_t> mask_dtheta;
    std::vector<float> osc_drift;
    std::vector<float> osc_step;
    std::vector<float> timing_rec;
    std::vector<float> fast_tab;
    float tw_s2[18];
    int init(int Fs, int Rs, int M, int P, int Nsym, int est_min, int est_max,
             int freq_est_type, int tone_spacing, int in_format, const pirip_fsk_recalled *recalled = nullptr);
};

struct FskMod {
    int Fs, Rs, M, Ts, f1_tx, tone_spacing;
    float ph_re = 1.0f, ph_im = 0.0f;
    void init(int Fs_, int Rs_, int M_, int f1, int spacing);
    void mod(const uint8_t *bits, int nbits, float *out, bool complex_out);
};

void test_frame_bits(uint8_t *frame, int framesize);

struct PutBits {
    int framesize; float valid_thresh;
    std::vector<uint8_t> tx, rx;
    long bitcnt = 0, biterr = 0; int packetcnt = 0;
    void init(int framesize_, float valid_thresh_);
    bool push(uint8_t bit, int *errs_out);
    float ber() const { return bitcnt ? (float)biterr / (float)bitcnt : 0.5f; }
};

int csdr_filter_len(float transition_bw);
void csdr_lowpass_hamming(float *taps, int length, float cutoff_rate);
void csdr_lowpass(float *taps, int length, float cutoff_rate, int window);
bool fsk_est_range(int Fs, int Ndft, int est_min, int est_max, int *st, int *en);
void recalled_defaults(pirip_fsk_recalled *r);
bool recalled_from_env(pirip_fsk_recalled *r);

}
```

pirip_amd/csrc/pirip_capi.hip:

```cpp
#include <hip/hip_runtime.h>

#include <cstdio>
#include <cstdlib>
#include <cstring>
#include <new>
#include <vector>

#include "../../include/pirip_hip.h"
#include "fsk_device.hpp"
#include "fsk_plan.hpp"
#include "demod_handle.hpp"

using namespace pirip;

#define HIPCHK(expr)                                              \
    do {                                                          \
        hipError_t e_ = (expr);                                   \
        if (e_ != hipSuccess) {                                   \
            h->last_hip = (int)e_;                                \
            return PIRIP_ERR_HIP;                                 \
        }                                                         \
    } while (0)


namespace {

int bytes_per_sample(int fmt)
{
    switch (fmt) {
    case PIRIP_IN_CU8_FSKDEMOD: case PIRIP_IN_CU8_CSDR: return 2;
    case PIRIP_IN_CS16: return 4;
    default: return 8;
    }
}

template <typename T>
hipError_t upload(T **dst, const void *src, size_t bytes)
{
    hipError_t e = hipMalloc((void **)dst, bytes ? bytes : 16);
    if (e != hipSuccess) return e;
    if (bytes) e = hipMemcpy(*dst, src, bytes, hipMemcpyHostToDevice);
    return e;
}

void free_all(pirip_hip_demod *h)
{
    void *ptrs[] = {h->d_hann, h->d_tw, h->d_perm, h->d_lut, h->d_tph, h->d_teeth, h->d_mask_dtheta,
                    h->d_osc_drift, h->d_osc_step, h->d_timing_rec, h->d_fast_tab,
                    h->d_Sf, h->d_theta, h->d_hist, h->d_scal, h->d_phic, h->d_first, h->d_stage_in, h->d_stage_bits,
                    h->d_stage_filt, h->d_stage_stats, h->d_stage_nframes, h->d_stage_consumed, h->d_eye};
    for (void *p : ptrs) if (p) (void)hipFree(p);
}

int reset_state(pirip_hip_demod *h, hipStream_t st)
{
    const FskDims &d = h->plan.d;
    const size_t ns = (size_t)h->nstreams;
    HIPCHK(hipMemsetAsync(h->d_Sf, 0, sizeof(float) * ns * d.Ndft, st));
    HIPCHK(hipMemsetAsync(h->d_theta, 0, sizeof(uint32_t) * ns * kMaxTones, st));
    HIPCHK(hipMemsetAsync(h->d_hist, 0, sizeof(float2) * ns * d.M * d.hist_len, st));
    HIPCHK(hipMemsetAsync(h->d_phic, 0, sizeof(float2) * ns * kMaxTones, st));
    std::vector<StreamScalars> sc(ns);
    std::memset(sc.data(), 0, sizeof(StreamScalars) * ns);
    for (auto &s : sc) s.nin = d.N;
    HIPCHK(hipMemcpyAsync(h->d_scal, sc.data(), sizeof(StreamScalars) * ns, hipMemcpyHostToDevice, st));
    HIPCHK(hipStreamSynchronize(st));
    h->nin0 = d.N;
    h->fresh = true;
    return PIRIP_OK;
}

void fill_args(const pirip_hip_demod *h, DemodArgs *a)
{
    a->d = h->plan.d;
    for (int i = 0; i < kMaxStages; i++) a->stages[i] = h->plan.stages[i];
    a->t = DemodTables{h->d_hann, h->d_tw, h->d_perm, h->d_lut, h->d_tph, h->d_teeth, h->d_mask_dtheta,
                       h->d_osc_drift, h->d_osc_step, h->d_timing_rec, h->d_fast_tab};
    for (int i = 0; i < 18; i++) a->tw_s2[i] = h->plan.tw_s2[i];
    a->s = DemodState{h->d_Sf, h->d_theta, h->d_hist, h->d_scal, h->d_phic};
}

bool bind(const pirip_hip_demod *h)
{
    int cur = -1;
    if (hipGetDevice(&cur) == hipSuccess && cur == h->device) return true;
    return hipSetDevice(h->device) == hipSuccess;
}

}

namespace pirip {
void demod_fill_args(const pirip_hip_demod *h, DemodArgs *a) { fill_args(h, a); }
bool demod_bind(const pirip_hip_demod *h) { return bind(h); }
void capture_release(pirip_hip_demod *h);
}

extern "C" {

const char *pirip_hip_version(void) { return "pirip_hip 0.2 (gfx950)"; }

int pirip_hip_abi(int *abi_version, int *stats_per_frame, size_t *stream_state_bytes)
{
    if (abi_version) *abi_version = PIRIP_HIP_ABI_VERSION;
    if (stats_per_frame) *stats_per_frame = PIRIP_STATS_PER_FRAME;
    if (stream_state_bytes) *stream_state_bytes = sizeof(pirip_stream_state);
    return PIRIP_OK;
}

int pirip_hip_abi_check(int abi_version, int stats_per_frame, size_t stream_state_bytes)
{
    return abi_version == PIRIP_HIP_ABI_VERSION && stats_per_frame == PIRIP_STATS_PER_FRAME && stream_state_bytes == sizeof(pirip_stream_state);
}

const char *pirip_hip_kernel_source_hash(void) { return pirip::demod_wave_source_hash(); }

const char *pirip_hip_strerror(int status)
{
    switch (status) {
    case PIRIP_OK: return "ok";
    case PIRIP_ERR_BAD_ARG: return "bad argument";
    case PIRIP_ERR_BAD_CONFIG: return "bad modem configuration (codec2 fsk_create would assert)";
    case PIRIP_ERR_NO_DEVICE: return "no usable HIP device";
    case PIRIP_ERR_HIP: return "HIP runtime error";
    case PIRIP_ERR_NOMEM: return "out of memory";
    case PIRIP_ERR_UNSUPPORTED: return "unsupported";
    default: return "unknown";
    }
}

int pirip_hip_device_count(void)
{
    int n = 0;
    if (hipGetDeviceCount(&n) != hipSuccess) return 0;
    return n;
}

int pirip_hip_selftest_atan2(const float *d_y, const float *d_x, float *d_out, int n)
{
    if (!d_y || !d_x || !d_out || n < 0) return PIRIP_ERR_BAD_ARG;
    if (pirip_hip_device_count() <= 0) return PIRIP_ERR_NO_DEVICE;
    return selftest_atan2(d_y, d_x, d_out, n) == hipSuccess ? PIRIP_OK : PIRIP_ERR_HIP;
}

int pirip_hip_selftest_sqrt(uint64_t *mismatches)
{
    if (!mismatches) return PIRIP_ERR_BAD_ARG;
    if (pirip_hip_device_count() <= 0) return PIRIP_ERR_NO_DEVICE;
    unsigned long long m = 0;
    if (selftest_sqrt(&m) != hipSuccess) return PIRIP_ERR_HIP;
    *mismatches = m;
    return PIRIP_OK;
}

int pirip_hip_selftest_div(uint64_t *mismatches)
{
    if (!mismatches) return PIRIP_ERR_BAD_ARG;
    if (pirip_hip_device_count() <= 0) return PIRIP_ERR_NO_DEVICE;
    unsigned long long m = 0;
    if (selftest_div(&m) != hipSuccess) return PIRIP_ERR_HIP;
    *mismatches = m;
    return PIRIP_OK;
}

static int est_band_for(pirip_hip_demod *h);
void pirip_hip_recalled_defaults(pirip_fsk_recalled *r) { if (r) recalled_defaults(r); }

int pirip_hip_create(const pirip_fsk_params *p, int nstreams, int device, pirip_hip_demod **out)
{
    return pirip_hip_create_recalled(p, nullptr, nstreams, device, out);
}

int pirip_hip_create_recalled(const pirip_fsk_params *p, const pirip_fsk_recalled *recalled, int nstreams, int device, pirip_hip_demod **out)
{
    if (!p || !out || nstreams <= 0) return PIRIP_ERR_BAD_ARG;
    *out = nullptr;
    pirip_hip_demod *h = new (std::nothrow) pirip_hip_demod();
    if (!h) return PIRIP_ERR_NOMEM;
    pirip_fsk_recalled from_env;
    if (!recalled && getenv("PIRIP_RECALLED")) {
        recalled_defaults(&from_env);
        if (!recalled_from_env(&from_env)) { delete h; return PIRIP_ERR_BAD_CONFIG; }
        recalled = &from_env;
    }
    int rc = h->plan.init(p->Fs, p->Rs, p->M, p->P, p->Nsym, p->est_min, p->est_max,
                          p->freq_est_type, p->tone_spacing, p->in_format, recalled);
    if (rc != PIRIP_OK) { delete h; return rc; }
    if (demod_general_lds_bytes(h->plan.d) > 160 * 1024) { delete h; return PIRIP_ERR_UNSUPPORTED; }

    int ndev = pirip_hip_device_count();
    if (ndev <= 0) { delete h; return PIRIP_ERR_NO_DEVICE; }
    if (device >= 0) { if (device >= ndev || hipSetDevice(device) != hipSuccess) { delete h; return PIRIP_ERR_NO_DEVICE; } }
    if (hipGetDevice(&h->device) != hipSuccess) { delete h; return PIRIP_ERR_NO_DEVICE; }
    h->nstreams = nstreams;
    {
        const char *k = getenv("PIRIP_KERNEL");
        const bool want_general = getenv("PIRIP_FORCE_GENERAL") || (k && !strcmp(k, "general"));
        if (const char *f = getenv("PIRIP_FFT_FMA")) {
            h->plan.d.fft_fma = atoi(f) ? 1 : 0;
            if (h->plan.d.fft_fma && !demod_wave_applicable(h->plan.d)) h->plan.d.fft_fma = 0;
        }
        h->kernel = want_general || !h->plan.d.recalled_fast_ok ? 0 :
                    demod_wave_applicable(h->plan.d) ? PIRIP_KERNEL_WAVE : demod_block_applicable(h->plan.d) ? PIRIP_KERNEL_BLOCK : 0;
        if (const char *sg = getenv("PIRIP_BLOCK_STAGGER")) h->plan.d.block_stagger = atoi(sg) > 0 ? atoi(sg) : 0;
        if (const char *b = getenv("PIRIP_EST_BAND")) {
            if (atoi(b)) h->plan.d.est_band = est_band_for(h);
        }
        if (k && !strcmp(k, "exact")) {
            h->plan.d.grp = 1;
            if (!demod_exact_applicable(h->plan.d)) { delete h; return PIRIP_ERR_UNSUPPORTED; }
            h->kernel = PIRIP_KERNEL_EXACT;
        }
    }

    const FskPlan &pl = h->plan;
    const FskDims &d = pl.d;
    const size_t ns = (size_t)nstreams;
    bool ok = true;
    ok &= upload(&h->d_hann, pl.hann.data(), sizeof(float) * d.Ndft) == hipSuccess;
    ok &= upload(&h->d_tw, pl.twiddle.data(), sizeof(float) * 2 * d.Ndft) == hipSuccess;
    ok &= upload(&h->d_perm, pl.leaf_iperm.data(), sizeof(uint16_t) * d.Ndft) == hipSuccess;
    ok &= upload(&h->d_lut, pl.u8_lut.data(), sizeof(float) * 256) == hipSuccess;
    ok &= upload(&h->d_tph, pl.timing_ph.data(), sizeof(float) * 2 * d.P) == hipSuccess;
    ok &= upload(&h->d_teeth, pl.teeth.data(), sizeof(int16_t) * pl.teeth.size()) == hipSuccess;
    ok &= upload(&h->d_mask_dtheta, pl.mask_dtheta.data(), sizeof(uint32_t) * pl.mask_dtheta.size()) == hipSuccess;
    ok &= upload(&h->d_osc_drift, pl.osc_drift.data(), sizeof(float) * pl.osc_drift.size()) == hipSuccess;
    ok &= upload(&h->d_osc_step, pl.osc_step.data(), sizeof(float) * pl.osc_step.size()) == hipSuccess;
    ok &= upload(&h->d_timing_rec, pl.timing_rec.data(), sizeof(float) * pl.timing_rec.size()) == hipSuccess;
    ok &= upload(&h->d_fast_tab, pl.fast_tab.data(), sizeof(float) * pl.fast_tab.size()) == hipSuccess;
    ok &= hipMalloc((void **)&h->d_Sf, sizeof(float) * ns * d.Ndft) == hipSuccess;
    ok &= hipMalloc((void **)&h->d_theta, sizeof(uint32_t) * ns * kMaxTones) == hipSuccess;
    ok &= hipMalloc((void **)&h->d_hist, sizeof(float2) * ns * d.M * d.hist_len) == hipSuccess;
    ok &= hipMalloc((void **)&h->d_scal, sizeof(StreamScalars) * ns) == hipSuccess;
    ok &= hipMalloc((void **)&h->d_first, sizeof(int32_t) * ns) == hipSuccess;
    ok &= hipMalloc((void **)&h->d_phic, sizeof(float2) * ns * kMaxTones) == hipSuccess;
    if (!ok) { free_all(h); delete h; return PIRIP_ERR_NOMEM; }
    if (const char *e = getenv("PIRIP_EXACT0")) h->exact0 = atoi(e) ? 1 : 0;
    rc = reset_state(h, nullptr);
    if (rc != PIRIP_OK) { free_all(h); delete h; return rc; }
    *out = h;
    return PIRIP_OK;
}

int pirip_hip_destroy(pirip_hip_demod *h)
{
    if (!h) return PIRIP_ERR_BAD_ARG;
    (void)bind(h);
    (void)hipDeviceSynchronize();
    pirip::capture_release(h);
    free_all(h);
    delete h;
    return PIRIP_OK;
}

int pirip_hip_get_kernel(const pirip_hip_demod *h) { return h ? h->kernel : PIRIP_ERR_BAD_ARG; }

int pirip_hip_get_kernel_name(const pirip_hip_demod *h, char *buf, size_t n)
{
    if (!h || !buf || !n) return PIRIP_ERR_BAD_ARG;
    buf[0] = 0;
    if (h->kernel == 2 && demod_wave_describe(h->plan.d, buf, n) > 0) return PIRIP_OK;
    if (h->kernel == PIRIP_KERNEL_BLOCK && demod_block_describe(h->plan.d, buf, n) > 0) return PIRIP_OK;
    const FskDims &d = h->plan.d;
    snprintf(buf, n, "fsk_demod_%s_kernel(M=%d,Ts=%d,P=%d,Nsym=%d,Ndft=%d,format %d%s)", h->kernel == PIRIP_KERNEL_EXACT ? "exact" : "general", d.M, d.Ts, d.P, d.Nsym, d.Ndft, d.in_format,
             d.freq_est_type ? ",mask estimator" : "");
    return PIRIP_OK;
}

int pirip_hip_clear_estimators(pirip_hip_demod *h, void *hip_stream)
{
    if (!h) return PIRIP_ERR_BAD_ARG;
    if (!bind(h)) return PIRIP_ERR_NO_DEVICE;
    hipStream_t st = (hipStream_t)hip_stream;
    const FskDims &d = h->plan.d;
    const size_t ns = (size_t)h->nstreams;
    HIPCHK(hipMemsetAsync(h->d_Sf, 0, sizeof(float) * ns * d.Ndft, st));
    std::vector<int32_t> nin(ns, d.N);
    HIPCHK(hipMemcpy2DAsync(&h->d_scal->nin, sizeof(StreamScalars), nin.data(), sizeof(int32_t), sizeof(int32_t), ns, hipMemcpyHostToDevice, st));
    HIPCHK(hipStreamSynchronize(st));
    h->nin0 = d.N;
    return PIRIP_OK;
}

int pirip_hip_get_info(const pirip_hip_demod *h, pirip_fsk_info *info)
{
    if (!h || !info) return PIRIP_ERR_BAD_ARG;
    const FskDims &d = h->plan.d;
    info->Ts = d.Ts; info->N = d.N; info->Nmem = d.Nmem; info->Ndft = d.Ndft; info->Nbits = d.Nbits;
    info->nin_max = d.N + d.nin_step; info->nstreams = h->nstreams;
    info->bytes_per_sample = bytes_per_sample(d.in_format);
    return PIRIP_OK;
}

int pirip_hip_reset(pirip_hip_demod *h, void *hip_stream)
{
    if (!h) return PIRIP_ERR_BAD_ARG;
    if (!bind(h)) return PIRIP_ERR_NO_DEVICE;
    return reset_state(h, (hipStream_t)hip_stream);
}

}

namespace pirip {
int exact0_prologue(pirip_hip_demod *h, DemodArgs *a, hipStream_t st)
{
    const FskDims &d = h->plan.d;
    if (!h->fresh) return PIRIP_OK;
    if (a->io.nsamp < d.N || a->io.max_frames < 1) return PIRIP_OK;
    h->fresh = false;
    if (!h->exact0 || !demod_exact0_applicable(d) || h->kernel == PIRIP_KERNEL_BLOCK || h->kernel == PIRIP_KERNEL_EXACT || a->io.soft.llr || a->io.seg) return PIRIP_OK;
    DemodArgs p = *a;
    p.io.first = nullptr; p.io.first_out = h->d_first;
    p.io.exact0_fmt = h->kernel == PIRIP_KERNEL_WAVE ? PIRIP_KERNEL_WAVE : PIRIP_KERNEL_GENERAL;
    p.io.eye = h->d_eye;
    const hipError_t e = launch_demod_exact0(p, h->nstreams, st);
    if (e != hipSuccess) { h->last_hip = (int)e; return PIRIP_ERR_HIP; }
    a->io.first = h->d_first;
    return PIRIP_OK;
}
}

extern "C" {

int pirip_hip_set_exact_first_frame(pirip_hip_demod *h, int enable)
{
    if (!h) return PIRIP_ERR_BAD_ARG;
    h->exact0 = enable ? 1 : 0;
    return PIRIP_OK;
}

int pirip_hip_demod_batch(pirip_hip_demod *h, const void *d_in, size_t in_stride_bytes, int64_t nsamp,
                          uint8_t *d_bits, size_t bits_stride, float *d_rx_filt, size_t filt_stride,
                          float *d_stats, size_t stats_stride, int32_t *d_nframes, int64_t *d_consumed,
                          int64_t max_frames, void *hip_stream)
{
    return pirip::demod_batch_seg(h, d_in, in_stride_bytes, nsamp, d_bits, bits_stride, d_rx_filt, filt_stride, d_stats, stats_stride,
                                  d_nframes, d_consumed, max_frames, nullptr, (hipStream_t)hip_stream);
}

}

namespace pirip {
int demod_batch_seg(pirip_hip_demod *h, const void *d_in, size_t in_stride_bytes, int64_t nsamp,
                    uint8_t *d_bits, size_t bits_stride, float *d_rx_filt, size_t filt_stride,
                    float *d_stats, size_t stats_stride, int32_t *d_nframes, int64_t *d_consumed,
                    int64_t max_frames, const SegDesc *seg, hipStream_t hip_stream)
{
    if (!h || !d_in || nsamp < 0 || max_frames < 0) return PIRIP_ERR_BAD_ARG;
    if (!bind(h)) return PIRIP_ERR_NO_DEVICE;
    DemodArgs a;
    fill_args(h, &a);
    a.io = DemodIO{(const uint8_t *)d_in, in_stride_bytes, nsamp, d_bits, bits_stride, d_rx_filt, filt_stride,
                   d_stats, stats_stride, d_nframes, d_consumed, max_frames, SoftOut{nullptr, 0, nullptr, 0, nullptr, 0}};
    a.io.seg = seg;
    a.io.eye = (h->kernel == PIRIP_KERNEL_GENERAL || h->kernel == PIRIP_KERNEL_EXACT) ? h->d_eye : nullptr;
    hipError_t e;
    if (h->kernel == 2 && nsamp > demod_wave_max_samples(a.d)) return PIRIP_ERR_UNSUPPORTED;
    {
        const int pr = exact0_prologue(h, &a, (hipStream_t)hip_stream);
        if (pr != PIRIP_OK) return pr;
    }
    if (h->kernel == 2) {
        e = launch_demod_wave(a, h->nstreams, (hipStream_t)hip_stream);
    } else e = launch_demod_kind(h->kernel, a, h->nstreams, (hipStream_t)hip_stream);
    if (e != hipSuccess) { h->last_hip = (int)e; return PIRIP_ERR_HIP; }
    return PIRIP_OK;
}

int demod_batch_soft(pirip_hip_demod *h, const void *d_in, size_t in_stride_bytes, int64_t nsamp, const SoftOut &so, float *d_stats, size_t stats_stride,
                     int32_t *d_nframes, int64_t *d_consumed, int64_t max_frames, hipStream_t st, int s0, int n, const SegDesc *seg)
{
    if (!h || !d_in || nsamp < 0 || max_frames < 0 || !so.llr || !so.words || !so.lnI0 || (so.bit0 & 31)) return PIRIP_ERR_BAD_ARG;
    if (h->kernel != 2 || !demod_wave_soft_capable(h->plan.d) || nsamp > demod_wave_max_samples(h->plan.d)) return PIRIP_ERR_UNSUPPORTED;
    if (!bind(h)) return PIRIP_ERR_NO_DEVICE;
    DemodArgs a;
    fill_args(h, &a);
    a.io = DemodIO{(const uint8_t *)d_in, in_stride_bytes, nsamp, nullptr, 0, nullptr, 0, d_stats, stats_stride, d_nframes, d_consumed, max_frames, so};
    a.io.seg = seg;
    (void)exact0_prologue(h, &a, st);
    int nrun = h->nstreams;
    if (n >= 0) {
        if (s0 < 0 || s0 + n > h->nstreams) return PIRIP_ERR_BAD_ARG;
        const FskDims &d = h->plan.d;
        const size_t z = (size_t)s0;
        a.s.Sf += z * d.Ndft; a.s.theta += z * kMaxTones; a.s.hist += z * d.M * d.hist_len; a.s.scal += z;
        if (a.s.phic) a.s.phic += z * kMaxTones;
        a.io.in += z * in_stride_bytes;
        if (a.io.stats) a.io.stats += z * stats_stride;
        a.io.nframes += z;
        if (a.io.consumed) a.io.consumed += z;
        if (a.io.seg) a.io.seg += z;
        a.io.soft.llr += z * so.llr_stride; a.io.soft.words += z * so.words_stride;
        nrun = n;
    }
    if (nrun == 0) return PIRIP_OK;
    const hipError_t e = launch_demod_wave(a, nrun, st);
    if (e != hipSuccess) { h->last_hip = (int)e; return PIRIP_ERR_HIP; }
    return PIRIP_OK;
}
bool demod_soft_capable(const pirip_hip_demod *h, int64_t nsamp)
{
    return h && h->kernel == 2 && demod_wave_soft_capable(h->plan.d) && nsamp <= demod_wave_max_samples(h->plan.d);
}
int demod_streams_per_cu(const pirip_hip_demod *h) { return h && h->kernel == 2 ? demod_wave_streams_per_cu(h->plan.d) : 0; }
int demod_handle_shape(const pirip_hip_demod *h, int *M, int *Nsym, int *nstreams, int *device)
{
    if (!h) return PIRIP_ERR_BAD_ARG;
    *M = h->plan.d.M; *Nsym = h->plan.d.Nsym; *nstreams = h->nstreams; *device = h->device;
    return PIRIP_OK;
}
}

extern "C" {

int pirip_hip_demod_host(pirip_hip_demod *h, const void *in, int64_t nsamp, uint8_t *bits, float *rx_filt,
                         float *stats, int64_t max_frames, int64_t *nframes, int64_t *consumed)
{
    if (!h || (!in && nsamp > 0) || nsamp < 0 || max_frames < 0) return PIRIP_ERR_BAD_ARG;
    if (h->nstreams != 1) return PIRIP_ERR_BAD_ARG;
    if (!bind(h)) return PIRIP_ERR_NO_DEVICE;
    const FskDims &d = h->plan.d;
    const size_t bps = (size_t)bytes_per_sample(d.in_format);
    const size_t in_bytes = (size_t)nsamp * bps;
    if (in_bytes > h->stage_in_bytes) {
        if (h->d_stage_in) (void)hipFree(h->d_stage_in);
        h->d_stage_in = nullptr; h->stage_in_bytes = 0;
        HIPCHK(hipMalloc(&h->d_stage_in, in_bytes + 64));
        h->stage_in_bytes = in_bytes;
    }
    if (!h->d_stage_in) { HIPCHK(hipMalloc(&h->d_stage_in, 64)); h->stage_in_bytes = 0; }
    if (max_frames > h->stage_frames) {
        void *olds[] = {h->d_stage_bits, h->d_stage_filt, h->d_stage_stats};
        for (void *p : olds) if (p) (void)hipFree(p);
        h->d_stage_bits = nullptr; h->d_stage_filt = nullptr; h->d_stage_stats = nullptr; h->stage_frames = 0;
        HIPCHK(hipMalloc((void **)&h->d_stage_bits, (size_t)max_frames * d.Nbits + 16));
        HIPCHK(hipMalloc((void **)&h->d_stage_filt, sizeof(float) * (size_t)max_frames * d.M * d.Nsym + 16));
        HIPCHK(hipMalloc((void **)&h->d_stage_stats, sizeof(float) * (size_t)max_frames * PIRIP_STATS_PER_FRAME + 16));
        h->stage_frames = max_frames;
    }
    if (!h->d_stage_nframes) {
        HIPCHK(hipMalloc((void **)&h->d_stage_nframes, sizeof(int32_t) * (size_t)h->nstreams));
        HIPCHK(hipMalloc((void **)&h->d_stage_consumed, sizeof(int64_t) * (size_t)h->nstreams));
    }
    if (in_bytes) HIPCHK(hipMemcpy(h->d_stage_in, in, in_bytes, hipMemcpyHostToDevice));
    int rc = pirip_hip_demod_batch(h, h->d_stage_in, 0, nsamp, h->d_stage_bits, 0,
                                   rx_filt ? h->d_stage_filt : nullptr, 0,
                                   h->d_stage_stats, 0, h->d_stage_nframes, h->d_stage_consumed,
                                   max_frames, nullptr);
    if (rc != PIRIP_OK) return rc;
    HIPCHK(hipDeviceSynchronize());
    int32_t nf = 0; int64_t cons = 0;
    HIPCHK(hipMemcpy(&nf, h->d_stage_nframes, sizeof(nf), hipMemcpyDeviceToHost));
    HIPCHK(hipMemcpy(&cons, h->d_stage_consumed, sizeof(cons), hipMemcpyDeviceToHost));
    const size_t fb = d.pack_bits ? (size_t)(d.Nbits + 7) / 8 : (size_t)d.Nbits;
    if (bits && nf) HIPCHK(hipMemcpy(bits, h->d_stage_bits, (size_t)nf * fb, hipMemcpyDeviceToHost));
    if (rx_filt && nf) HIPCHK(hipMemcpy(rx_filt, h->d_stage_filt, sizeof(float) * (size_t)nf * d.M * d.Nsym, hipMemcpyDeviceToHost));
    if (stats && nf) HIPCHK(hipMemcpy(stats, h->d_stage_stats, sizeof(float) * (size_t)nf * PIRIP_STATS_PER_FRAME, hipMemcpyDeviceToHost));
    StreamScalars sc;
    HIPCHK(hipMemcpy(&sc, h->d_scal, sizeof(sc), hipMemcpyDeviceToHost));
    h->nin0 = sc.nin;
    if (nframes) *nframes = nf;
    if (consumed) *consumed = cons;
    return PIRIP_OK;
}

int pirip_hip_nin0(pirip_hip_demod *h) { return h ? h->nin0 : PIRIP_ERR_BAD_ARG; }

int pirip_hip_get_Sf(pirip_hip_demod *h, int s, float *Sf_host)
{
    if (!h || !Sf_host || s < 0 || s >= h->nstreams) return PIRIP_ERR_BAD_ARG;
    if (!bind(h)) return PIRIP_ERR_NO_DEVICE;
    HIPCHK(hipDeviceSynchronize());
    HIPCHK(hipMemcpy(Sf_host, h->d_Sf + (size_t)s * h->plan.d.Ndft, sizeof(float) * h->plan.d.Ndft, hipMemcpyDeviceToHost));
    return PIRIP_OK;
}

int pirip_hip_enable_eye(pirip_hip_demod *h, int enable)
{
    if (!h) return PIRIP_ERR_BAD_ARG;
    if (!bind(h)) return PIRIP_ERR_NO_DEVICE;
    HIPCHK(hipDeviceSynchronize());
    if (!enable) {
        if (h->d_eye) (void)hipFree(h->d_eye);
        h->d_eye = nullptr;
        return PIRIP_OK;
    }
    if (h->d_eye) return PIRIP_OK;
    const size_t bytes = sizeof(float) * (size_t)h->nstreams * kEyeTraces * kEyePoints;
    HIPCHK(hipMalloc((void **)&h->d_eye, bytes));
    HIPCHK(hipMemset(h->d_eye, 0, bytes));
    if (h->kernel != PIRIP_KERNEL_GENERAL && h->kernel != PIRIP_KERNEL_EXACT) {
        h->kernel = PIRIP_KERNEL_GENERAL;
        return reset_state(h, nullptr);
    }
    return PIRIP_OK;
}

int pirip_hip_get_eye(pirip_hip_demod *h, int s, int normalise, float *rx_eye, int *neyetr, int *neyesamp)
{
    if (!h || !rx_eye || !neyetr || !neyesamp || s < 0 || s >= h->nstreams) return PIRIP_ERR_BAD_ARG;
    if (!h->d_eye) return PIRIP_ERR_UNSUPPORTED;
    if (!bind(h)) return PIRIP_ERR_NO_DEVICE;
    HIPCHK(hipDeviceSynchronize());
    HIPCHK(hipMemcpy(rx_eye, h->d_eye + (size_t)s * kEyeTraces * kEyePoints, sizeof(float) * kEyeTraces * kEyePoints, hipMemcpyDeviceToHost));
    const FskDims &d = h->plan.d;
    const int dec = (2 * d.P + kEyePoints - 1) / kEyePoints, npts = (2 * d.P) / dec;
    int traces = kEyeTraces / d.M;
    while (traces > 0 && 2 * d.P * traces + (d.P / 2 + 1) + (npts - 1) * dec >= (d.Nsym + 1) * d.P) traces--;
    if (normalise) {
        float eye_max = 0.f;
        for (int i = 0; i < traces * d.M; i++)
            for (int j = 0; j < npts; j++) if (fabsf(rx_eye[i * kEyePoints + j]) > eye_max) eye_max = fabsf(rx_eye[i * kEyePoints + j]);
        if (eye_max > 0.f)
            for (int i = 0; i < traces * d.M; i++)
                for (int j = 0; j < npts; j++) rx_eye[i * kEyePoints + j] = rx_eye[i * kEyePoints + j] / eye_max;
    }
    *neyetr = traces * d.M; *neyesamp = npts;
    return PIRIP_OK;
}

int pirip_hip_set_bit_packing(pirip_hip_demod *h, int packed)
{
    if (!h) return PIRIP_ERR_BAD_ARG;
    h->plan.d.pack_bits = packed ? 1 : 0;
    return PIRIP_OK;
}

static int est_band_for(pirip_hip_demod *h)
{
    pirip::FskDims d = h->plan.d;
    if (h->kernel != PIRIP_KERNEL_WAVE || d.freq_est_type != 0 || d.Ndft != 256 || d.est_st < d.Ndft / 2) return 0;
    for (int b = 2; b <= 4; b += 2) {
        d.est_band = b;
        if (d.est_en <= d.Ndft / 2 + 16 * b && demod_wave_applicable(d)) return b;
    }
    return 0;
}
int pirip_hip_set_estimator_band_only(pirip_hip_demod *h, int enable)
{
    if (!h) return PIRIP_ERR_BAD_ARG;
    if (enable) {
        const int b = est_band_for(h);
        if (!b) return PIRIP_ERR_UNSUPPORTED;
        h->plan.d.est_band = b;
        return PIRIP_OK;
    }
    if (!h->plan.d.est_band) return PIRIP_OK;
    h->plan.d.est_band = 0;
    return pirip_hip_reset(h, nullptr);
}

int pirip_hip_set_burst_mode(pirip_hip_demod *h, int enable)
{
    if (!h) return PIRIP_ERR_BAD_ARG;
    h->plan.d.burst_mode = enable ? 1 : 0;
    if (enable) {
        if (!bind(h)) return PIRIP_ERR_NO_DEVICE;
        HIPCHK(hipDeviceSynchronize());
        std::vector<StreamScalars> sc((size_t)h->nstreams);
        HIPCHK(hipMemcpy(sc.data(), h->d_scal, sizeof(StreamScalars) * sc.size(), hipMemcpyDeviceToHost));
        for (auto &s : sc) s.nin = h->plan.d.N;
        HIPCHK(hipMemcpy(h->d_scal, sc.data(), sizeof(StreamScalars) * sc.size(), hipMemcpyHostToDevice));
        h->nin0 = h->plan.d.N;
    }
    return PIRIP_OK;
}

int pirip_hip_get_scalars(pirip_hip_demod *h, int s, float *out8)
{
    if (!h || !out8 || s < 0 || s >= h->nstreams) return PIRIP_ERR_BAD_ARG;
    if (!bind(h)) return PIRIP_ERR_NO_DEVICE;
    HIPCHK(hipDeviceSynchronize());
    StreamScalars sc;
    HIPCHK(hipMemcpy(&sc, h->d_scal + s, sizeof(sc), hipMemcpyDeviceToHost));
    out8[0] = sc.f_est[0]; out8[1] = sc.f_est[1]; out8[2] = sc.f_est[2]; out8[3] = sc.f_est[3];
    out8[4] = sc.norm_rx_timing; out8[5] = sc.SNRest; out8[6] = (float)sc.nin; out8[7] = sc.ppm;
    return PIRIP_OK;
}

int pirip_hip_get_stream_state(pirip_hip_demod *h, int s, pirip_stream_state *out)
{
    if (!h || !out || s < 0 || s >= h->nstreams) return PIRIP_ERR_BAD_ARG;
    if (!bind(h)) return PIRIP_ERR_NO_DEVICE;
    HIPCHK(hipDeviceSynchronize());
    StreamScalars sc;
    HIPCHK(hipMemcpy(&sc, h->d_scal + s, sizeof(sc), hipMemcpyDeviceToHost));
    out->nin = sc.nin; out->norm_rx_timing = sc.norm_rx_timing; out->ppm = sc.ppm; out->snr_est = sc.snr_est;
    out->SNRest = sc.SNRest; out->EbNodB = sc.EbNodB; out->v_est = sc.v_est;
    for (int m = 0; m < 4; m++) out->f_est[m] = sc.f_est[m];
    out->rx_sig_pow = sc.rx_sig_pow; out->rx_nse_pow = sc.rx_nse_pow;
    return PIRIP_OK;
}

int pirip_hip_set_freq_est_limits(pirip_hip_demod *h, int est_min, int est_max)
{
    if (!h) return PIRIP_ERR_BAD_ARG;
    int st, en;
    if (!fsk_est_range(h->plan.d.Fs, h->plan.d.Ndft, est_min, est_max, &st, &en)) return PIRIP_ERR_BAD_CONFIG;
    if (h->plan.d.est_band && (st < h->plan.d.Ndft / 2 || en > h->plan.d.Ndft / 2 + 16 * h->plan.d.est_band)) return PIRIP_ERR_UNSUPPORTED;
    h->plan.d.est_st = st; h->plan.d.est_en = en;
    return PIRIP_OK;
}

}
```

Before: 342,000 IQ Msamples/s.

## Run band-only estimator speculatively with full-spectrum catch-up and per-stream redo

Makes an automatic estimator mode the default for the wave kernel. Most of each stream is demodulated with the cheaper band-only frequency estimator. A catch-up pass then runs the last 64 frames with both the band-only and a shadow full-spectrum smoothed spectrum, and checks that the results match bit for bit. Streams that diverge are flagged, and a redo kernel reprocesses them from snapshotted state (Sf, history, scalars) using the full estimator. This aims to cut the cost of computing and smoothing all 256 DFT bins, at the price of extra device-to-device snapshot copies, two extra kernel launches, and full reprocessing of any stream that fails the check.

```diff
diff --git a/include/pirip_hip.h b/include/pirip_hip.h
--- a/include/pirip_hip.h
+++ b/include/pirip_hip.h
@@ -104,6 +104,9 @@
 int pirip_hip_set_bit_packing(pirip_hip_demod *h, int packed);
 
 int pirip_hip_set_estimator_band_only(pirip_hip_demod *h, int enable);
+
+int pirip_hip_set_estimator_auto(pirip_hip_demod *h, int enable);
+int pirip_hip_get_estimator_auto_counters(pirip_hip_demod *h, uint64_t *calls, uint64_t *streams_redone, int32_t *redo_host);
 
 int pirip_hip_set_burst_mode(pirip_hip_demod *h, int enable);
 
diff --git a/pirip_amd/binding.py b/pirip_amd/binding.py
--- a/pirip_amd/binding.py
+++ b/pirip_amd/binding.py
@@ -273,6 +273,19 @@
     def set_estimator_band_only(self, enable=True):
         _chk(self.L.pirip_hip_set_estimator_band_only(self.h, 1 if enable else 0), "pirip_hip_set_estimator_band_only")
 
+    def set_estimator_auto(self, enable=True):
+        self.L.pirip_hip_set_estimator_auto.argtypes = [C.c_void_p, C.c_int]
+        _chk(self.L.pirip_hip_set_estimator_auto(self.h, 1 if enable else 0), "pirip_hip_set_estimator_auto")
+
+    def estimator_auto_counters(self):
+        import numpy as np
+        calls, redone = C.c_uint64(0), C.c_uint64(0)
+        hold = np.zeros(self.nstreams, dtype=np.int32)
+        self.L.pirip_hip_get_estimator_auto_counters.argtypes = [C.c_void_p, C.c_void_p, C.c_void_p, C.c_void_p]
+        _chk(self.L.pirip_hip_get_estimator_auto_counters(self.h, C.byref(calls), C.byref(redone), hold.ctypes.data),
+             "pirip_hip_get_estimator_auto_counters")
+        return calls.value, redone.value, hold
+
     def set_freq_est_limits(self, est_min, est_max):
         return int(self.L.pirip_hip_set_freq_est_limits(self.h, int(est_min), int(est_max)))
 
diff --git a/pirip_amd/csrc/demod_handle.hpp b/pirip_amd/csrc/demod_handle.hpp
--- a/pirip_amd/csrc/demod_handle.hpp
+++ b/pirip_amd/csrc/demod_handle.hpp
@@ -25,10 +25,17 @@
     int exact0 = 1;
     int32_t *d_first = nullptr;
     float *d_eye = nullptr;
+    int est_auto = 1;
+    int32_t *d_redo = nullptr;
+    float *d_Sf0 = nullptr; float2 *d_hist0 = nullptr; pirip::StreamScalars *d_scal0 = nullptr;
+    int64_t *d_apos = nullptr; int32_t *d_aframe = nullptr;
+    unsigned *d_redo_count = nullptr;
+    uint64_t est_auto_calls = 0;
     struct CaptureWork *capture = nullptr;
 };
 
 namespace pirip {
+constexpr int kEstCatchupFrames = 64;
 void demod_fill_args(const pirip_hip_demod *h, DemodArgs *a);
 bool demod_bind(const pirip_hip_demod *h);
 }
diff --git a/pirip_amd/csrc/fsk_demod_wave.hip b/pirip_amd/csrc/fsk_demod_wave.hip
--- a/pirip_amd/csrc/fsk_demod_wave.hip
+++ b/pirip_amd/csrc/fsk_demod_wave.hip
@@ -204,7 +204,7 @@
 
 }
 
-template <int M, int TS, int P, int NSYM, int NDFT, int FMT, int WPB, int WPS, bool FFT_FMA = false, bool MASK = false, int BAND = 0>
+template <int M, int TS, int P, int NSYM, int NDFT, int FMT, int WPB, int WPS, bool FFT_FMA = false, bool MASK = false, int BAND = 0, int EMODE = 0>
 __global__ __launch_bounds__(kWave * WPB, WPS) void fsk_demod_wave_kernel(DemodArgs a_kernarg, int nstreams)
 {
     constexpr bool INPLACE = TS == 10;
@@ -217,6 +217,7 @@
 #define a (*ap)
 #define d (ap->d)
     static_assert(BAND == 0 || ((BAND == 2 || BAND == 4) && NDFT == 256 && !MASK), "band-only estimator: Ndft = 256, peak method, 32 or 64 bins");
+    static_assert(EMODE == 0 || (BAND == 0 && NDFT == 256 && !MASK && P > 10 && FMT != PIRIP_IN_CF32), "catch-up / redo: full estimator, Ndft = 256, bounded input, no fused hand-over");
     auto cmul = [](v2f x, v2f t) { return FFT_FMA ? rot_step(x, t) : cmul_x(x, t); };
     using C = WaveCfg<M, TS, P, NSYM, NDFT, FMT>;
     constexpr int N = C::N, NMEM = C::NMEM, HIST = C::HIST, STEP = C::STEP, Q = C::Q, BPS = C::BPS;
@@ -256,20 +257,23 @@
     __syncthreads();
     if (sid >= nstreams) return;
     if (a.io.seg && a.io.seg[sid].max_frames < 0) return;
+    if constexpr (EMODE == 0) { if (a.au.redo && a.au.redo[sid] > 0) return; }
+    else if ((a.au.redo[sid] > 0) != (EMODE == 2)) return;
 
     unsigned char *raw = s_raw[wv];
     unsigned char *xpb = s_xp[wv];
 
     uint32_t *st32 = (uint32_t *)(a.s.hist + (size_t)sid * M * HIST);
-    int ninp = __builtin_amdgcn_readfirstlane((int)st32[C::TRAILER_DW + 2 * M]);
+    const uint32_t *st32_in = EMODE == 2 ? (const uint32_t *)(a.au.hist0 + (size_t)sid * M * HIST) : st32;
+    int ninp = __builtin_amdgcn_readfirstlane((int)st32_in[C::TRAILER_DW + 2 * M]);
     uint32_t dthp[M];
     int tixp[M];
 #pragma unroll
     for (int m = 0; m < M; m++) {
-        dthp[m] = (uint32_t)__builtin_amdgcn_readfirstlane((int)st32[C::TRAILER_DW + m]);
-        tixp[m] = __builtin_amdgcn_readfirstlane((int)st32[C::TRAILER_DW + M + m]);
-    }
-    for (int i = lane0; i < GUARD_B / 4; i += kWave) ((uint32_t *)raw)[i] = ninp ? st32[i] : InFmt<FMT>::NEUTRAL;
+        dthp[m] = (uint32_t)__builtin_amdgcn_readfirstlane((int)st32_in[C::TRAILER_DW + m]);
+        tixp[m] = __builtin_amdgcn_readfirstlane((int)st32_in[C::TRAILER_DW + M + m]);
+    }
+    for (int i = lane0; i < GUARD_B / 4; i += kWave) ((uint32_t *)raw)[i] = ninp ? st32_in[i] : InFmt<FMT>::NEUTRAL;
 
 #define PIRIP_PHASE_LANE(name) int name = lane0; asm volatile("" : "+v"(name))
     constexpr int NOWN = NDFT / kWave;
@@ -290,12 +294,21 @@
         for (int i = 0; i < 16; i++) hann16[i] = a.t.fast_tab[(lane0 & 7) + 8 * i];
     }
 #pragma unroll
-    for (int b = 0; b < NB; b++) Sf[b] = a.s.Sf[(size_t)sid * NDFT + own_sfi(lane0, b)];
+    for (int b = 0; b < NB; b++) Sf[b] = (EMODE == 2 ? a.au.Sf0 : a.s.Sf)[(size_t)sid * NDFT + own_sfi(lane0, b)];
+    float Sh[EMODE == 1 ? NOWN : 1];
+    if constexpr (EMODE == 1) {
+#pragma unroll
+        for (int b = 0; b < NOWN; b++) {
+            const bool inband = lane0 < 16 && b < 2;
+            Sh[b] = inband ? Sf[b] : a.au.sf_max;
+            Sf[b] = inband ? Sf[b] : 0.0f;
+        }
+    }
 
     float sc_norm_rx_timing, sc_ppm, sc_SNRest;
     int sc_nin;
     {
-        const StreamScalars sc = a.s.scal[sid];
+        const StreamScalars sc = (EMODE == 2 ? a.au.scal0 : a.s.scal)[sid];
         sc_norm_rx_timing = sc.norm_rx_timing; sc_ppm = sc.ppm; sc_SNRest = sc.SNRest; sc_nin = sc.nin;
         if (lane0 == 0) { s_misc[wv][0] = sc.snr_est; s_misc[wv][1] = sc.EbNodB; s_misc[wv][2] = sc.v_est; }
     }
@@ -313,6 +326,11 @@
     int nin = __builtin_amdgcn_readfirstlane(sc_nin);
     int64_t pos = 0, frame = 0;
     if (a.io.first) { pos = __builtin_amdgcn_readfirstlane(a.io.first[sid]); frame = pos ? 1 : 0; }
+    if constexpr (EMODE == 1) {
+        const int64_t p = a.au.pos[sid];
+        pos = ((int64_t)__builtin_amdgcn_readfirstlane((int)(p >> 32)) << 32) | (uint32_t)__builtin_amdgcn_readfirstlane((int)(uint32_t)p);
+        frame = __builtin_amdgcn_readfirstlane(a.au.frame[sid]);
+    }
     const int64_t frame_first = frame;
     int last_freqi0 = 0, last_freqi1 = 0, last_freqi2 = 0, last_freqi3 = 0;
 
@@ -531,6 +549,17 @@
                         }
                         Sf[0] = s01.x; Sf[1] = s01.y; Sf[2] = s23.x; Sf[3] = s23.y;
                     }
+                    if constexpr (EMODE == 1) {
+                        v2f h01{Sh[0], Sh[1]}, h23{Sh[2], Sh[3]};
+#pragma unroll
+                        for (int g2 = 0; g2 < 4; g2++) {
+                            if (C::NFFT % 4 == 0 || 4 * bt + g2 < C::NFFT) {
+                                h01 = smooth2(h01, v2f{rt[g2].x, rt[g2].y}, ktc);
+                                h23 = smooth2(h23, v2f{rt[g2].z, rt[g2].w}, ktc);
+                            }
+                        }
+                        Sh[0] = h01.x; Sh[1] = h01.y; Sh[2] = h23.x; Sh[3] = h23.y;
+                    }
                     wave_lds_sync();
                 }
             }
@@ -1188,6 +1217,16 @@
     if (a.io.stats && lane0 == 0 && sid == nstreams / 2)
         for (int i = 0; i < 8; i++) a.io.stats[(size_t)sid * a.io.stats_stride + i] = (float)t_acc_[i];
 #endif
+    if constexpr (EMODE == 1) {
+        bool same = true;
+#pragma unroll
+        for (int b = 0; b < NOWN; b++) same = same && fbits(Sf[b]) == fbits(Sh[b]);
+        if (!__all(same)) {
+            if (lane0 == 0) a.au.redo[sid] = kEstRedoHold;
+            return;
+        }
+    }
+    if constexpr (EMODE == 2) if (lane0 == 0) { a.au.redo[sid] = a.au.redo[sid] - 1; atomicAdd(a.au.count, 1u); }
 #pragma unroll
     for (int b = 0; b < NB; b++) if (!BAND || lane0 < 16) a.s.Sf[(size_t)sid * NDFT + own_sfi(lane0, b)] = Sf[b];
     wave_lds_sync();
@@ -1285,11 +1324,11 @@
 namespace {
 
 struct WaveInst {
-    int M, Ts, P, Nsym, Ndft, fmt, fft_fma, mask, wpb, wps, band;
+    int M, Ts, P, Nsym, Ndft, fmt, fft_fma, mask, wpb, wps, band, emode;
     hipError_t (*launch)(const DemodArgs &, int, hipStream_t);
 };
 
-template <int M, int TS, int P, int NSYM, int NDFT, int FMT, int WPB, int WPS, bool FMA, bool MASK, int BAND = 0>
+template <int M, int TS, int P, int NSYM, int NDFT, int FMT, int WPB, int WPS, bool FMA, bool MASK, int BAND = 0, int EMODE = 0>
 hipError_t launch_inst(const DemodArgs &a, int nstreams, hipStream_t stream)
 {
     const dim3 g((nstreams + WPB - 1) / WPB), b(kWave * WPB);
@@ -1302,19 +1341,22 @@
         (void)hipStreamSynchronize(stream);
     }
 #endif
-    hipLaunchKernelGGL((fsk_demod_wave_kernel<M, TS, P, NSYM, NDFT, FMT, WPB, WPS, FMA, MASK, BAND>), g, b, dyn, stream, a, nstreams);
+    hipLaunchKernelGGL((fsk_demod_wave_kernel<M, TS, P, NSYM, NDFT, FMT, WPB, WPS, FMA, MASK, BAND, EMODE>), g, b, dyn, stream, a, nstreams);
     return hipGetLastError();
 }
 
-#define PIRIP_WAVE_INST(M, TS, P, NDFT, FMT, WPB, WPS) {M, TS, P, 50, NDFT, FMT, 0, 0, WPB, WPS, 0, launch_inst<M, TS, P, 50, NDFT, FMT, WPB, WPS, false, false>}
-#define PIRIP_WAVE_INST_FMA(M, TS, P, NDFT, FMT, WPB, WPS) {M, TS, P, 50, NDFT, FMT, 1, 0, WPB, WPS, 0, launch_inst<M, TS, P, 50, NDFT, FMT, WPB, WPS, true, false>}
-#define PIRIP_WAVE_INST_MASK(M, TS, P, NDFT, FMT, WPB, WPS) {M, TS, P, 50, NDFT, FMT, 0, 1, WPB, WPS, 0, launch_inst<M, TS, P, 50, NDFT, FMT, WPB, WPS, false, true>}
-#define PIRIP_WAVE_INST_BAND(M, TS, P, NDFT, FMT, WPB, WPS, B) {M, TS, P, 50, NDFT, FMT, 0, 0, WPB, WPS, B, launch_inst<M, TS, P, 50, NDFT, FMT, WPB, WPS, false, false, B>}
+#define PIRIP_WAVE_INST(M, TS, P, NDFT, FMT, WPB, WPS) {M, TS, P, 50, NDFT, FMT, 0, 0, WPB, WPS, 0, 0, launch_inst<M, TS, P, 50, NDFT, FMT, WPB, WPS, false, false>}
+#define PIRIP_WAVE_INST_FMA(M, TS, P, NDFT, FMT, WPB, WPS) {M, TS, P, 50, NDFT, FMT, 1, 0, WPB, WPS, 0, 0, launch_inst<M, TS, P, 50, NDFT, FMT, WPB, WPS, true, false>}
+#define PIRIP_WAVE_INST_MASK(M, TS, P, NDFT, FMT, WPB, WPS) {M, TS, P, 50, NDFT, FMT, 0, 1, WPB, WPS, 0, 0, launch_inst<M, TS, P, 50, NDFT, FMT, WPB, WPS, false, true>}
+#define PIRIP_WAVE_INST_BAND(M, TS, P, NDFT, FMT, WPB, WPS, B) {M, TS, P, 50, NDFT, FMT, 0, 0, WPB, WPS, B, 0, launch_inst<M, TS, P, 50, NDFT, FMT, WPB, WPS, false, false, B>}
+#define PIRIP_WAVE_INST_EST(M, TS, P, NDFT, FMT, WPB, WPS, E) {M, TS, P, 50, NDFT, FMT, 0, 0, WPB, WPS, 0, E, launch_inst<M, TS, P, 50, NDFT, FMT, WPB, WPS, false, false, 0, E>}
 const WaveInst kInst[] = {
     PIRIP_WAVE_INST(2, 24, 24, 256, PIRIP_IN_CU8_FSKDEMOD, 4, 3),
     PIRIP_WAVE_INST_FMA(2, 24, 24, 256, PIRIP_IN_CU8_FSKDEMOD, 4, 3),
     PIRIP_WAVE_INST(2, 24, 24, 256, PIRIP_IN_CU8_CSDR, 4, 3),
     PIRIP_WAVE_INST_BAND(2, 24, 24, 256, PIRIP_IN_CU8_FSKDEMOD, 4, 3, 2), PIRIP_WAVE_INST_BAND(2, 24, 24, 256, PIRIP_IN_CU8_CSDR, 4, 3, 2),
+    PIRIP_WAVE_INST_EST(2, 24, 24, 256, PIRIP_IN_CU8_FSKDEMOD, 4, 3, 1), PIRIP_WAVE_INST_EST(2, 24, 24, 256, PIRIP_IN_CU8_FSKDEMOD, 4, 3, 2),
+    PIRIP_WAVE_INST_EST(2, 24, 24, 256, PIRIP_IN_CU8_CSDR, 4, 3, 1), PIRIP_WAVE_INST_EST(2, 24, 24, 256, PIRIP_IN_CU8_CSDR, 4, 3, 2),
     PIRIP_WAVE_INST_BAND(4, 24, 8, 256, PIRIP_IN_CU8_FSKDEMOD, 4, 3, 4), PIRIP_WAVE_INST_BAND(4, 24, 8, 256, PIRIP_IN_CU8_CSDR, 4, 3, 4),
 #define PIRIP_TS24(M, P, WPB, WPS) \
     PIRIP_WAVE_INST(M, 24, P, 256, PIRIP_IN_CU8_FSKDEMOD, WPB, WPS), PIRIP_WAVE_INST(M, 24, P, 256, PIRIP_IN_CU8_CSDR, WPB, WPS), \
@@ -1339,13 +1381,14 @@
 #undef PIRIP_WAVE_INST_FMA
 #undef PIRIP_WAVE_INST_MASK
 #undef PIRIP_WAVE_INST_BAND
-
-const WaveInst *find_inst(const FskDims &d)
+#undef PIRIP_WAVE_INST_EST
+
+const WaveInst *find_inst(const FskDims &d, int emode = 0)
 {
     if (!d.recalled_fast_ok) return nullptr;
     for (const WaveInst &w : kInst)
         if (w.M == d.M && w.Ts == d.Ts && w.P == d.P && w.Nsym == d.Nsym && w.Ndft == d.Ndft && w.fmt == d.in_format && w.fft_fma == d.fft_fma &&
-            w.mask == (d.freq_est_type != 0) && w.band == d.est_band) return &w;
+            w.mask == (d.freq_est_type != 0) && w.band == d.est_band && w.emode == emode) return &w;
     return nullptr;
 }
 
@@ -1372,11 +1415,21 @@
     return 0x7fffff00LL / bps * 2 / 2;
 }
 
-hipError_t launch_demod_wave(const DemodArgs &a, int nstreams, hipStream_t stream)
-{
-    const WaveInst *w = find_inst(a.d);
+hipError_t launch_demod_wave_est(const DemodArgs &a, int nstreams, hipStream_t stream, int est_mode)
+{
+    const WaveInst *w = find_inst(a.d, est_mode);
     if (!w || a.io.nsamp > demod_wave_max_samples(a.d)) return hipErrorNotSupported;
     return w->launch(a, nstreams, stream);
 }
 
-}
+hipError_t launch_demod_wave(const DemodArgs &a, int nstreams, hipStream_t stream) { return launch_demod_wave_est(a, nstreams, stream, 0); }
+
+int demod_wave_auto_band(const FskDims &d)
+{
+    if (d.est_band || !find_inst(d, 0) || !find_inst(d, 1) || !find_inst(d, 2)) return 0;
+    FskDims b = d;
+    b.est_band = 2;
+    return find_inst(b, 0) ? 2 : 0;
+}
+
+}
diff --git a/pirip_amd/csrc/fsk_device.hpp b/pirip_amd/csrc/fsk_device.hpp
--- a/pirip_amd/csrc/fsk_device.hpp
+++ b/pirip_amd/csrc/fsk_device.hpp
@@ -100,6 +100,18 @@
     int exact0_fmt;
 };
 
+constexpr int kEstRedoHold = 4;
+struct EstAuto {
+    int32_t *redo;
+    const float *Sf0;
+    const float2 *hist0;
+    const StreamScalars *scal0;
+    const int64_t *pos;
+    const int32_t *frame;
+    unsigned *count;
+    float sf_max;
+};
+
 struct DemodArgs {
     FskDims d;
     FftStage stages[kMaxStages];
@@ -107,6 +119,7 @@
     DemodState s;
     DemodIO io;
     float tw_s2[18];
+    EstAuto au;
 };
 
 int demod_batch_seg(pirip_hip_demod *h, const void *d_in, size_t in_stride_bytes, int64_t nsamp, uint8_t *d_bits, size_t bits_stride,
@@ -136,6 +149,8 @@
 bool demod_wave_soft_capable(const FskDims &d);
 int64_t demod_wave_max_samples(const FskDims &d);
 hipError_t launch_demod_wave(const DemodArgs &a, int nstreams, hipStream_t stream);
+int demod_wave_auto_band(const FskDims &d);
+hipError_t launch_demod_wave_est(const DemodArgs &a, int nstreams, hipStream_t stream, int est_mode);
 bool demod_block_applicable(const FskDims &d);
 int demod_block_describe(const FskDims &d, char *buf, size_t n);
 hipError_t launch_demod_block(const DemodArgs &a, int nstreams, hipStream_t stream);
diff --git a/pirip_amd/csrc/fsk_plan.cpp b/pirip_amd/csrc/fsk_plan.cpp
--- a/pirip_amd/csrc/fsk_plan.cpp
+++ b/pirip_amd/csrc/fsk_plan.cpp
@@ -202,6 +202,13 @@
     }
     fast_tab.clear();
     for (auto &v : tw_s2) v = 0.f;
+    {
+        double hsum = 0.0, xmax = 0.0;
+        for (float v : hann) hsum += std::fabs((double)v);
+        if (in_format == PIRIP_IN_CS16) xmax = 32768.0 / (double)rc.s16_scale;
+        else if (in_format != PIRIP_IN_CF32) for (float v : u8_lut) xmax = std::fabs((double)v) > xmax ? std::fabs((double)v) : xmax;
+        sf_max = (float)(1.0625 * hsum * std::sqrt(2.0) * xmax);
+    }
     if (Ndft == 256) {
         fast_tab.assign(16 * 48, 0.f);
         for (int e = 0; e < 16; e++) {
diff --git a/pirip_amd/csrc/fsk_plan.hpp b/pirip_amd/csrc/fsk_plan.hpp
--- a/pirip_amd/csrc/fsk_plan.hpp
+++ b/pirip_amd/csrc/fsk_plan.hpp
@@ -54,6 +54,7 @@
     std::vector<float> timing_rec;
     std::vector<float> fast_tab;
     float tw_s2[18];
+    float sf_max = 0.0f;
     int init(int Fs, int Rs, int M, int P, int Nsym, int est_min, int est_max,
              int freq_est_type, int tone_spacing, int in_format, const pirip_fsk_recalled *recalled = nullptr);
 };
diff --git a/pirip_amd/csrc/pirip_capi.hip b/pirip_amd/csrc/pirip_capi.hip
--- a/pirip_amd/csrc/pirip_capi.hip
+++ b/pirip_amd/csrc/pirip_capi.hip
@@ -48,7 +48,8 @@
     void *ptrs[] = {h->d_hann, h->d_tw, h->d_perm, h->d_lut, h->d_tph, h->d_teeth, h->d_mask_dtheta,
                     h->d_osc_drift, h->d_osc_step, h->d_timing_rec, h->d_fast_tab,
                     h->d_Sf, h->d_theta, h->d_hist, h->d_scal, h->d_phic, h->d_first, h->d_stage_in, h->d_stage_bits,
-                    h->d_stage_filt, h->d_stage_stats, h->d_stage_nframes, h->d_stage_consumed, h->d_eye};
+                    h->d_stage_filt, h->d_stage_stats, h->d_stage_nframes, h->d_stage_consumed, h->d_eye,
+                    h->d_redo, h->d_Sf0, h->d_hist0, h->d_scal0, h->d_apos, h->d_aframe, h->d_redo_count};
     for (void *p : ptrs) if (p) (void)hipFree(p);
 }
 
@@ -78,6 +79,65 @@
                        h->d_osc_drift, h->d_osc_step, h->d_timing_rec, h->d_fast_tab};
     for (int i = 0; i < 18; i++) a->tw_s2[i] = h->plan.tw_s2[i];
     a->s = DemodState{h->d_Sf, h->d_theta, h->d_hist, h->d_scal, h->d_phic};
+    a->au = EstAuto{};
+}
+
+int est_auto_band(const pirip_hip_demod *h)
+{
+    const FskDims &d = h->plan.d;
+    if (!h->est_auto || h->kernel != PIRIP_KERNEL_WAVE || d.est_band || d.fft_fma || !(h->plan.sf_max > 0.0f)) return 0;
+    const int b = demod_wave_auto_band(d);
+    if (!b || d.est_st < d.Ndft / 2 || d.est_en > d.Ndft / 2 + 16 * b) return 0;
+    return b;
+}
+
+int est_auto_alloc(pirip_hip_demod *h)
+{
+    if (h->d_redo) return PIRIP_OK;
+    const FskDims &d = h->plan.d;
+    const size_t ns = (size_t)h->nstreams;
+    bool ok = true;
+    ok &= hipMalloc((void **)&h->d_Sf0, sizeof(float) * ns * d.Ndft) == hipSuccess;
+    ok &= hipMalloc((void **)&h->d_hist0, sizeof(float2) * ns * d.M * d.hist_len) == hipSuccess;
+    ok &= hipMalloc((void **)&h->d_scal0, sizeof(StreamScalars) * ns) == hipSuccess;
+    ok &= hipMalloc((void **)&h->d_apos, sizeof(int64_t) * ns) == hipSuccess;
+    ok &= hipMalloc((void **)&h->d_aframe, sizeof(int32_t) * ns) == hipSuccess;
+    ok &= hipMalloc((void **)&h->d_redo_count, sizeof(unsigned)) == hipSuccess;
+    ok &= hipMalloc((void **)&h->d_redo, sizeof(int32_t) * ns) == hipSuccess;
+    if (ok) ok = hipMemset(h->d_redo, 0, sizeof(int32_t) * ns) == hipSuccess && hipMemset(h->d_redo_count, 0, sizeof(unsigned)) == hipSuccess;
+    if (!ok) {
+        void *ptrs[] = {h->d_Sf0, h->d_hist0, h->d_scal0, h->d_apos, h->d_aframe, h->d_redo_count, h->d_redo};
+        for (void *p : ptrs) if (p) (void)hipFree(p);
+        h->d_Sf0 = nullptr; h->d_hist0 = nullptr; h->d_scal0 = nullptr; h->d_apos = nullptr; h->d_aframe = nullptr; h->d_redo_count = nullptr; h->d_redo = nullptr;
+        return PIRIP_ERR_NOMEM;
+    }
+    return PIRIP_OK;
+}
+
+hipError_t launch_est_auto(pirip_hip_demod *h, const DemodArgs &a, int band, hipStream_t st)
+{
+    const FskDims &d = h->plan.d;
+    const size_t ns = (size_t)h->nstreams;
+    const EstAuto au{h->d_redo, h->d_Sf0, h->d_hist0, h->d_scal0, h->d_apos, h->d_aframe, h->d_redo_count, h->plan.sf_max};
+    hipError_t e;
+    if ((e = hipMemcpyAsync(h->d_Sf0, h->d_Sf, sizeof(float) * ns * d.Ndft, hipMemcpyDeviceToDevice, st)) != hipSuccess) return e;
+    if ((e = hipMemcpyAsync(h->d_hist0, h->d_hist, sizeof(float2) * ns * d.M * d.hist_len, hipMemcpyDeviceToDevice, st)) != hipSuccess) return e;
+    if ((e = hipMemcpyAsync(h->d_scal0, h->d_scal, sizeof(StreamScalars) * ns, hipMemcpyDeviceToDevice, st)) != hipSuccess) return e;
+    DemodArgs x = a;
+    x.au = au;
+    x.d.est_band = band;
+    x.io.nsamp = a.io.nsamp - (int64_t)kEstCatchupFrames * (d.N + d.nin_step);
+    x.io.max_frames = a.io.max_frames - kEstCatchupFrames;
+    x.io.nframes = h->d_aframe; x.io.consumed = h->d_apos;
+    if ((e = launch_demod_wave_est(x, h->nstreams, st, 0)) != hipSuccess) return e;
+    x = a;
+    x.au = au;
+    x.io.first = nullptr;
+    if ((e = launch_demod_wave_est(x, h->nstreams, st, 1)) != hipSuccess) return e;
+    x.io.first = a.io.first;
+    if ((e = launch_demod_wave_est(x, h->nstreams, st, 2)) != hipSuccess) return e;
+    h->est_auto_calls++;
+    return hipSuccess;
 }
 
 bool bind(const pirip_hip_demod *h)
@@ -201,6 +261,7 @@
         }
         h->kernel = want_general || !h->plan.d.recalled_fast_ok ? 0 :
                     demod_wave_applicable(h->plan.d) ? PIRIP_KERNEL_WAVE : demod_block_applicable(h->plan.d) ? PIRIP_KERNEL_BLOCK : 0;
+        if (const char *ea = getenv("PIRIP_EST_AUTO")) h->est_auto = atoi(ea) ? 1 : 0;
         if (const char *sg = getenv("PIRIP_BLOCK_STAGGER")) h->plan.d.block_stagger = atoi(sg) > 0 ? atoi(sg) : 0;
         if (const char *b = getenv("PIRIP_EST_BAND")) {
             if (atoi(b)) h->plan.d.est_band = est_band_for(h);
@@ -258,7 +319,12 @@
 {
     if (!h || !buf || !n) return PIRIP_ERR_BAD_ARG;
     buf[0] = 0;
-    if (h->kernel == 2 && demod_wave_describe(h->plan.d, buf, n) > 0) return PIRIP_OK;
+    if (h->kernel == 2 && demod_wave_describe(h->plan.d, buf, n) > 0) {
+        const int b = est_auto_band(h);
+        const size_t l = strlen(buf);
+        if (b) snprintf(buf + l, n - l, "+BAND%d+catchup", b);
+        return PIRIP_OK;
+    }
     if (h->kernel == PIRIP_KERNEL_BLOCK && demod_block_describe(h->plan.d, buf, n) > 0) return PIRIP_OK;
     const FskDims &d = h->plan.d;
     snprintf(buf, n, "fsk_demod_%s_kernel(M=%d,Ts=%d,P=%d,Nsym=%d,Ndft=%d,format %d%s)", h->kernel == PIRIP_KERNEL_EXACT ? "exact" : "general", d.M, d.Ts, d.P, d.Nsym, d.Ndft, d.in_format,
@@ -360,7 +426,13 @@
         if (pr != PIRIP_OK) return pr;
     }
     if (h->kernel == 2) {
-        e = launch_demod_wave(a, h->nstreams, (hipStream_t)hip_stream);
+        const int band = seg ? 0 : est_auto_band(h);
+        const int64_t whole = nsamp / (a.d.N + a.d.nin_step) < max_frames ? nsamp / (a.d.N + a.d.nin_step) : max_frames;
+        if (band && whole >= 4 * kEstCatchupFrames) {
+            const int rc = est_auto_alloc(h);
+            if (rc != PIRIP_OK) return rc;
+            e = launch_est_auto(h, a, band, (hipStream_t)hip_stream);
+        } else e = launch_demod_wave(a, h->nstreams, (hipStream_t)hip_stream);
     } else e = launch_demod_kind(h->kernel, a, h->nstreams, (hipStream_t)hip_stream);
     if (e != hipSuccess) { h->last_hip = (int)e; return PIRIP_ERR_HIP; }
     return PIRIP_OK;
@@ -549,6 +621,29 @@
     return pirip_hip_reset(h, nullptr);
 }
 
+int pirip_hip_set_estimator_auto(pirip_hip_demod *h, int enable)
+{
+    if (!h) return PIRIP_ERR_BAD_ARG;
+    h->est_auto = enable ? 1 : 0;
+    return PIRIP_OK;
+}
+
+int pirip_hip_get_estimator_auto_counters(pirip_hip_demod *h, uint64_t *calls, uint64_t *streams_redone, int32_t *redo_host)
+{
+    if (!h) return PIRIP_ERR_BAD_ARG;
+    if (!bind(h)) return PIRIP_ERR_NO_DEVICE;
+    HIPCHK(hipDeviceSynchronize());
+    if (calls) *calls = h->est_auto_calls;
+    unsigned n = 0;
+    if (h->d_redo_count) HIPCHK(hipMemcpy(&n, h->d_redo_count, sizeof(n), hipMemcpyDeviceToHost));
+    if (streams_redone) *streams_redone = n;
+    if (redo_host) {
+        if (h->d_redo) HIPCHK(hipMemcpy(redo_host, h->d_redo, sizeof(int32_t) * (size_t)h->nstreams, hipMemcpyDeviceToHost));
+        else memset(redo_host, 0, sizeof(int32_t) * (size_t)h->nstreams);
+    }
+    return PIRIP_OK;
+}
+
 int pirip_hip_set_burst_mode(pirip_hip_demod *h, int enable)
 {
     if (!h) return PIRIP_ERR_BAD_ARG;
```

Result: slower. 244,200 IQ Msamples/s (-28.6%).
